# google/zopfli

Hardware: AMD Instinct MI355X
Metric: input MB/s at numiterations=15 (gzip, bit-exact vs reference) (higher is better)
Workload: dtype u8 (f32/f64 cost DP); 1 GPU; class-T synthetic (text-like, the enwik8 stand-in) 100000000 B per GPU, numiterations=15, blocksplitting=0, gzip, BASELINE configs[1]; total_bytes=100000000, master_blocks=100, gather=none (one rank)

## Files before the change

### zopfli_amd/csrc/device/drv_build.h

```cpp
#pragma once

constexpr u32 kMatchGrid = 1024;
constexpr u32 kMatchGrid5 = 1536;

extern "C" {
static unsigned SegL(u64 total_positions) {
  if (Knobs().seg_l_set) return Knobs().seg_l;
  return total_positions <= (128u << 10) ? 256u : total_positions <= (16u << 20) ? 512u : total_positions <= (48u << 20) ? 1024u : 2048u;
}
static unsigned SegHead(size_t nb) {
  const unsigned v = Knobs().seg_head;
  return v ? v : (nb >= 48 ? 8192u : 0u);
}


static int LayoutBlocks(zmx_ctx* c, const zmx_block* blocks, size_t nb, zmx_tables* t, u64* la_total, u64* max_window) {
  t->nb = nb;
  t->blocks.resize(nb);
  t->bsize.resize(nb);
  t->store_begin[0].assign(nb, 0);
  t->store_begin[1].assign(nb, 0);
  std::vector<u32> tile_off(nb + 1, 0);
  u64 pos_off = 0, reg_off = 0, la_off = 0, max_l = 0;
  for (size_t b = 0; b < nb; ++b) {
    if (blocks[b].inend < blocks[b].instart || blocks[b].inend > c->insize) {
      return FailMsg("zmx_tables_build: block outside the resident input");
    }
    BlockDesc& d = t->blocks[b];
    d.instart = blocks[b].instart;
    d.inend = blocks[b].inend;
    d.ws = d.instart > ZMX_WINDOW ? d.instart - ZMX_WINDOW : 0;
    if (!c->seg_starts.empty()) {
      const size_t k = static_cast<size_t>(std::upper_bound(c->seg_starts.begin(), c->seg_starts.end(), d.instart) -
                                           c->seg_starts.begin()) - 1;
      const u64 seg_end = k + 1 < c->seg_starts.size() ? c->seg_starts[k + 1] : c->insize;
      if (d.inend > seg_end) return FailMsg("zmx_tables_build: block spans two input segments (zmx_set_input_segments)");
      d.ws = std::max<u64>(d.ws, c->seg_starts[k]);
    }
    d.pos_off = pos_off;
    d.reg_off = reg_off;
    d.la_off = la_off;
    const u64 B = d.inend - d.instart, L = d.inend - d.ws;
    if (B > 0x7fff0000ull) return FailMsg("zmx_tables_build: block too large (positions are 32-bit)");
    t->bsize[b] = static_cast<u32>(B);
    pos_off += B;
    reg_off += (L + 7) & ~7ull;
    la_off += (B + 1 + 7) & ~7ull;
    max_l = std::max(max_l, L);
    tile_off[b + 1] = tile_off[b] + static_cast<u32>((B + MT - 1) / MT);
  }
  t->total_b = pos_off;
  t->total_l = reg_off;
  t->tile_off = tile_off;
  *la_total = la_off;
  *max_window = max_l;
  return 0;
}

struct ReusePlan {
  bool reuse = false;
  std::vector<u64> src_pos;
  std::vector<u64> link_lo;
  std::vector<u32> tile_list;
};
static ReusePlan PlanReuse(const zmx_ctx* c, const zmx_tables* t, const zmx_tables* parent, const std::vector<uint64_t>& tail_r) {
  const size_t nb = t->nb;
  const u64 pos_off = t->total_b;
  const std::vector<u32>& tile_off = t->tile_off;
  ReusePlan plan;
  bool reuse = parent != nullptr && parent->nb > 0 && (c->h_in != nullptr || tail_r.size() == nb) && parent->d_recs != nullptr &&
               parent->total_b + pos_off < (3ull << 30);
  if (reuse) {
    plan.src_pos.resize(nb);
    plan.link_lo.resize(nb);
    size_t pb = 0;
    for (size_t b = 0; b < nb && reuse; ++b) {
      const BlockDesc& d = t->blocks[b];
      while (pb < parent->nb && parent->blocks[pb].inend < d.inend) ++pb;
      if (pb == parent->nb || d.instart < parent->blocks[pb].instart || d.inend > parent->blocks[pb].inend) {
        reuse = false;
        break;
      }
      const BlockDesc& pd = parent->blocks[pb];
      plan.src_pos[b] = pd.pos_off + (d.instart - pd.instart);
      const u64 B = d.inend - d.instart;
      plan.link_lo[b] = d.inend - d.ws;
      if (B == 0 || d.inend == pd.inend) continue;
      u64 t0 = B > ZMX_MAX_MATCH ? d.inend - ZMX_MAX_MATCH : d.instart;
      const u64 r = c->h_in ? zamd::TailRunStart(c->h_in, d.instart, d.inend) : tail_r[b];
      if (r < t0) t0 = r;
      const u32 tile_first = static_cast<u32>((t0 - d.instart) / MT);
      for (u32 tile = tile_first; tile < tile_off[b + 1] - tile_off[b]; ++tile) {
        plan.tile_list.push_back(tile_off[b] + tile);
      }
      const u64 first_index = d.instart + static_cast<u64>(tile_first) * MT - d.ws;
      plan.link_lo[b] = first_index > ZMX_WINDOW ? first_index - ZMX_WINDOW : 0;
    }
  }
  plan.reuse = reuse;
  return plan;
}

static int TailRuns(zmx_ctx* c, const zmx_tables* t, std::vector<uint64_t>* r) {
  const size_t nb = t->nb;
  std::vector<uint64_t> blocks(2 * nb);
  for (size_t b = 0; b < nb; ++b) {
    blocks[2 * b] = t->blocks[b].instart;
    blocks[2 * b + 1] = t->blocks[b].inend;
  }
  PoolScope tmp(c);
  uint64_t* d_blocks = nullptr;
  uint64_t* d_r = nullptr;
  HIPCHK(tmp.Upload(&d_blocks, blocks.data(), 2 * nb, "d_blocks"));
  HIPCHK(tmp.AllocT(&d_r, nb, "d_r"));
  TailRunParams P;
  P.in = c->d_in;
  P.blocks = d_blocks;
  P.r = d_r;
  hipLaunchKernelGGL(k_tail_runs, dim3(static_cast<unsigned>(nb)), dim3(64), 0, c->stream, P);
  KCHK(c, "k_tail_runs");
  r->resize(nb);
  HIPCHK(hipMemcpyAsync(r->data(), d_r, nb * sizeof(uint64_t), hipMemcpyDeviceToHost, c->stream));
  HIPCHK(hipStreamSynchronize(c->stream));
  return 0;
}

static int AllocTableArrays(zmx_ctx* c, zmx_tables* t, u64 la_off) {
  const size_t nb = t->nb;
  const u64 pos_off = t->total_b;
  const u64 reg_off = t->total_l;
  const std::vector<u32>& tile_off = t->tile_off;
  HIPCHK(PoolAlloc(c, &t->d_blocks, nb));
  HIPCHK(PoolAlloc(c, &t->d_tile_off, nb + 1));
  HIPCHK(PoolAlloc(c, &t->d_same16, reg_off));
  HIPCHK(PoolAlloc(c, &t->d_links, reg_off));
  HIPCHK(PoolAlloc(c, &t->d_recs, pos_off * 8));
  HIPCHK(PoolAlloc(c, &t->d_la, la_off));
  HIPCHK(PoolAlloc(c, &t->d_store[0], pos_off));
  HIPCHK(PoolAlloc(c, &t->d_store[1], pos_off));
  t->run = RunLayout(nb);
  HIPCHK(PoolAlloc(c, &t->d_runin, t->run.in_bytes));
  HIPCHK(PoolAlloc(c, &t->d_runout, t->run.out_bytes));
  HIPCHK(c->pool.PinnedTake(&t->h_runin, t->run.in_bytes, &t->h_runin_cap));
  HIPCHK(c->pool.PinnedTake(&t->h_runout, t->run.out_bytes, &t->h_runout_cap));
  HIPCHK(hipMemsetAsync(t->run.stats(t->d_runout), 0, RunLayout::stats_and_flags_bytes(), c->stream));
  HIPCHK(PoolAlloc(c, &t->d_dph, pos_off));
  HIPCHK(PoolAlloc(c, &t->d_block_edges, nb));
  t->badpos_words = pos_off / 32 + 4;
  HIPCHK(PoolAlloc(c, &t->d_badpos, t->badpos_words));
  HIPCHK(PoolAlloc(c, &t->d_code_base, nb));
  HIPCHK(PoolAlloc(c, &t->d_wtab, nb * ZMX_WTAB));
  HIPCHK(PoolAlloc(c, &t->d_badcodes, nb * 40));
  HIPCHK(PoolAlloc(c, &t->d_counters, 48));
  HIPCHK(hipMemcpyAsync(t->d_blocks, t->blocks.data(), nb * sizeof(BlockDesc), hipMemcpyHostToDevice, c->stream));
  HIPCHK(hipMemcpyAsync(t->d_tile_off, tile_off.data(), (nb + 1) * sizeof(u32), hipMemcpyHostToDevice, c->stream));
  HIPCHK(hipMemsetAsync(t->run.flags(t->d_runout), 0, RunLayout::kFlags * sizeof(u32), c->stream));
  return 0;
}

struct MatchBuild {
// ... 231 lines not shown
    HIPCHK(hipMemsetAsync(t->d_counters, 0, 48 * sizeof(u32), c->stream));
    if (LaunchMatch(c, t, mk, m, t->d_pool, t->pool_cap, tile_off[nb], nullptr, Knobs().prof) != 0) return -1;
    u32 counters[2] = {0, 0};
    HIPCHK(hipMemcpyAsync(counters, t->d_counters, sizeof(counters), hipMemcpyDeviceToHost, c->stream));
    HIPCHK(hipStreamSynchronize(c->stream));
    match_positions += static_cast<double>(pos_off);
    if (m.d_m5stats) {
      const size_t m5_waves = static_cast<size_t>(kMatchGrid5) * (M5_THREADS / 64);
      std::vector<unsigned long long> ws(2 * m5_waves);
      HIPCHK(hipMemcpy(ws.data(), m.d_m5stats, ws.size() * sizeof(unsigned long long), hipMemcpyDeviceToHost));
      m5_lane_iters = m5_iters = 0;
      for (size_t w = 0; w < m5_waves; ++w) { m5_lane_iters += static_cast<double>(ws[2 * w]); m5_iters += static_cast<double>(ws[2 * w + 1]); }
    }
    if (counters[1] & 2u) {
      u32 dbg[8] = {0};
      HIPCHK(hipMemcpy(dbg, t->d_counters + 32, sizeof(dbg), hipMemcpyDeviceToHost));
      char buf[320];
      std::snprintf(buf, sizeof(buf), "zmx_tables_build: k_match5's wave loop did not end (state %08x xd %u curd %u bestlen %u limit %u nlink %u eqd %u "
                    "li %u idx %u same %u cur %u bestdist %u)", dbg[0], dbg[1], dbg[2], dbg[3] & 0xffffu, dbg[3] >> 16, dbg[4] & 0xffffu, dbg[4] >> 16,
                    dbg[5], dbg[6] & 0xffffu, dbg[6] >> 16, dbg[7] & 0xffffu, dbg[7] >> 16);
      return FailFault(buf);
    }
    if ((counters[1] & 1u) == 0) break;
    if (per_pos >= 256) return FailMsg("zmx_tables_build: change-point pool overflow");
    per_pos *= 8;
  }
  {
    HIPCHK(hipEventRecord(c->ev[2], c->stream));
    HIPCHK(hipEventSynchronize(c->ev[2]));
    float ms_hash = 0, ms_match = 0;
    HIPCHK(hipEventElapsedTime(&ms_hash, c->ev[0], c->ev[1]));
    HIPCHK(hipEventElapsedTime(&ms_match, c->ev[1], c->ev[2]));
    zmx_stats& ts = zamd::ThreadStats();
    ts.match[0] += ms_match * 1e-3;
    ts.match[1] += ms_hash * 1e-3;
    ts.match[2] += 1;
    ts.match[3] += reuse ? static_cast<double>(plan.tile_list.size()) * MT : match_positions;
    if (m.skip_any && !reuse) {
      ts.match5[0] += m5_lane_iters;
      ts.match5[1] += m5_iters;
      ts.match5[2] += m.skip_positions;
    }
    if (Knobs().prof && !reuse) {
      unsigned long long hc[2] = {0, 0};
      HIPCHK(hipMemcpy(hc, t->d_counters + 4, sizeof(hc), hipMemcpyDeviceToHost));
      const double pos = static_cast<double>(pos_off);
      std::fprintf(stderr, "%s: %.2f ms for %.0f positions: %.1f chain hits per "
                   "position, %.1f of 64 lanes with a hit per wave-loop iteration; %.1f SIMD cycles per hit (2.4 GHz, 1024 SIMDs)\n", mk == 5 || mk == 0 ? "k_match5 / k_match2 (hits = entries touched)" : "k_match2", ms_match, pos,
                   static_cast<double>(hc[0]) / pos, static_cast<double>(hc[0]) / static_cast<double>(hc[1] ? hc[1] : 1),
                   ms_match * 1e-3 * 2.4e9 * 1024 / static_cast<double>(hc[0] ? hc[0] : 1));
      if (mk != 5) {
        int wgs = 0;
        if (Knobs().match_filter) HIPCHK(hipOccupancyMaxActiveBlocksPerMultiprocessor(&wgs, k_match2<false, true>, M2_THREADS, 0));
        else HIPCHK(hipOccupancyMaxActiveBlocksPerMultiprocessor(&wgs, k_match2<false, false>, M2_THREADS, 0));
        std::fprintf(stderr, "k_match2: %d workgroups of %u threads resident per CU; positions handed out %s\n", wgs, M2_THREADS,
                     m.d_est ? "by k_hits' estimate, longest first" : "in ascending order");
      }
    }
  }
  return 0;
}

static int BuildDpRows(zmx_ctx* c, zmx_tables* t) {
  const size_t nb = t->nb;
  const std::vector<u32>& tile_off = t->tile_off;
  RowScanParams rp;
  rp.blocks = t->d_blocks;
  rp.recs = t->d_recs;
  rp.dph = t->d_dph;
  rp.block_edges = t->d_block_edges;
  rp.codeless = !Knobs().run_codes && SegL(t->total_b) != 0 ? 1u : 0u;
  hipLaunchKernelGGL(k_rowscan, dim3(static_cast<unsigned>(nb)), dim3(1024), 0, c->stream, rp);
  KCHK(c, "k_rowscan");
  t->block_edges.resize(nb);
  HIPCHK(hipMemcpyAsync(t->block_edges.data(), t->d_block_edges, nb * sizeof(u64), hipMemcpyDeviceToHost, c->stream));
  HIPCHK(hipStreamSynchronize(c->stream));
  {
    const u64 env_mb = Knobs().code_budget_mb;
    const u64 budget = (env_mb ? env_mb * (1ull << 20) : static_cast<u64>(c->code_budget)) / sizeof(u16);
    std::vector<u64> code_base(nb, 0);
    u64 cur = 0;
    for (size_t b = 0; b < nb; ++b) {
      if (t->block_edges[b] > 0xffff0000ull) return FailMsg("zmx_tables_build: block too large (DP row offsets are 32-bit)");
      code_base[b] = cur;
      cur += ((t->block_edges[b] + DP_PIECE - 1) & ~static_cast<u64>(DP_PIECE - 1)) + DP_PIECE;
    }
    if (cur > budget && nb > 1) {
      return FailTooLarge("zmx_tables_build: the batch needs more room for its DP edges than ZOPFLI_AMD_CODE_BUDGET_MB allows");
    }
    HIPCHK(PoolAlloc(c, &t->d_codes, cur + 2048));
    HIPCHK(hipMemcpyAsync(t->d_code_base, code_base.data(), nb * sizeof(u64), hipMemcpyHostToDevice, c->stream));
    CodeParams kp;
    kp.blocks = t->d_blocks;
    kp.tile_off = t->d_tile_off;
    kp.nb_total = static_cast<u32>(nb);
    kp.recs = t->d_recs;
    kp.pool = t->d_pool;
    kp.dph = t->d_dph;
    kp.codes = t->d_codes;
    kp.code_base = t->d_code_base;
    if (tile_off[nb]) hipLaunchKernelGGL(k_codes, dim3(tile_off[nb]), dim3(256), 0, c->stream, kp);
    KCHK(c, "k_codes");
    t->win_off.assign(nb + 1, 0);
    for (size_t b = 0; b < nb; ++b) t->win_off[b + 1] = t->win_off[b] + (t->bsize[b] + 31) / 32 + 1;
    HIPCHK(PoolAlloc(c, &t->d_winflag, t->win_off[nb]));
    HIPCHK(PoolAlloc(c, &t->d_winroff, t->win_off[nb]));
    HIPCHK(PoolAlloc(c, &t->d_wmeta, (static_cast<size_t>(t->win_off[nb]) + 2) * D5_WM));
    HIPCHK(PoolAlloc(c, &t->d_win_off, nb + 1));
    HIPCHK(hipMemcpyAsync(t->d_win_off, t->win_off.data(), (nb + 1) * sizeof(u32), hipMemcpyHostToDevice, c->stream));
    MkDescParams mp;
    mp.blocks = t->d_blocks;
    mp.dph = t->d_dph;
    mp.wmeta = t->d_wmeta;
    mp.winroff = t->d_winroff;
    mp.win_off = t->d_win_off;
    mp.winflag = t->d_winflag;
    u32 max_b = 1;
    for (size_t b = 0; b < nb; ++b) max_b = std::max(max_b, t->bsize[b]);
    hipLaunchKernelGGL(k_mkdesc, dim3((max_b + 255) / 256, static_cast<unsigned>(nb)), dim3(256), 0, c->stream, mp);
    KCHK(c, "k_mkdesc");
    HIPCHK(hipStreamSynchronize(c->stream));
  }
  return 0;
}

static int BuildChainTasks(zmx_ctx* c, zmx_tables* t) {
  const size_t nb = t->nb;
  const u32 L = SegL(t->total_b), warm = Knobs().seg_warm;
  const u32 head = std::max(SegHead(nb), L);
  t->task_off.assign(nb + 1, 0);
  t->tasks.clear();
  for (size_t b = 0; b < nb; ++b) {
    const u32 B = t->bsize[b];
    const u32 n = (L == 0 || B < head + L) ? 1u : 1u + (B - head) / L;
    for (u32 s = 0; s < n; ++s) {
      SegTask k;
      k.block = static_cast<u32>(b);
      k.pout = s == 0 ? 0u : head + (s - 1) * L;
      k.q = s == 0 ? 0u : k.pout - std::min(warm, k.pout);
      k.pend = s + 1 == n ? B + 1 : head + s * L;
      t->tasks.push_back(k);
    }
    t->task_off[b + 1] = static_cast<u32>(t->tasks.size());
  }
  const size_t nt = t->tasks.size();
  HIPCHK(PoolAlloc(c, &t->d_tasks, nt));
  HIPCHK(PoolAlloc(c, &t->d_task_off, nb + 1));
  HIPCHK(PoolAlloc(c, &t->d_lvl, nt));
  HIPCHK(PoolAlloc(c, &t->d_entry, nt));
  HIPCHK(PoolAlloc(c, &t->d_exit, nt));
  HIPCHK(PoolAlloc(c, &t->d_mid, nt));
  HIPCHK(PoolAlloc(c, &t->d_chk, nt));
  HIPCHK(PoolAlloc(c, &t->d_over, nt * SEG_OVER));
  HIPCHK(PoolAlloc(c, &t->d_redo, 4 + nt * 4));
  HIPCHK(hipMemcpyAsync(t->d_tasks, t->tasks.data(), nt * sizeof(SegTask), hipMemcpyHostToDevice, c->stream));
  HIPCHK(hipMemcpyAsync(t->d_task_off, t->task_off.data(), (nb + 1) * sizeof(u32), hipMemcpyHostToDevice, c->stream));
  HIPCHK(hipMemsetAsync(t->run.stats(t->d_runout), 0, RunLayout::kStats * sizeof(u32), c->stream));
  const u32 cut_depth = Knobs().seg_cuts;
  if (cut_depth && nt) {
    PoolScope tmp(c);
    u32* d_found = nullptr;
    u32* d_wide = nullptr;
    HIPCHK(tmp.AllocT(&d_found, 2, "d_found"));
    HIPCHK(tmp.AllocT(&d_wide, nt, "d_wide"));
    HIPCHK(hipMemsetAsync(d_found, 0, 2 * sizeof(u32), c->stream));
    HIPCHK(hipMemsetAsync(d_wide, 0, nt * sizeof(u32), c->stream));
    CutParams cp;
    cp.blocks = t->d_blocks;
    cp.dph = t->d_dph;
    cp.tasks = t->d_tasks;
    cp.depth = cut_depth;
    cp.warm = warm;
    cp.found = d_found;
    cp.wide = d_wide;
    hipLaunchKernelGGL(k_cutpoints, dim3(static_cast<unsigned>(nt)), dim3(64), 0, c->stream, cp);
    KCHK(c, "k_cutpoints");
    u32 found[2] = {0, 0};
    std::vector<u32> wide(nt);
    HIPCHK(hipMemcpyAsync(found, d_found, sizeof(found), hipMemcpyDeviceToHost, c->stream));
    HIPCHK(hipMemcpyAsync(wide.data(), d_wide, nt * sizeof(u32), hipMemcpyDeviceToHost, c->stream));
    HIPCHK(hipMemcpyAsync(t->tasks.data(), t->d_tasks, nt * sizeof(SegTask), hipMemcpyDeviceToHost, c->stream));
    HIPCHK(hipStreamSynchronize(c->stream));
    size_t merged = 0;
    std::vector<SegTask> kept;
    kept.reserve(nt);
    std::vector<u32> off(nb + 1, 0);
    for (size_t b = 0; b < nb; ++b) {
      for (u32 k = t->task_off[b]; k < t->task_off[b + 1]; ++k) {
        if (k > t->task_off[b] && wide[k]) {
          kept.back().pend = t->tasks[k].pend;
          ++merged;
        } else {
          kept.push_back(t->tasks[k]);
        }
      }
      off[b + 1] = static_cast<u32>(kept.size());
    }
    t->merged_tasks = merged;
    if (merged) {
      t->tasks.swap(kept);
      t->task_off.swap(off);
      HIPCHK(hipMemcpyAsync(t->d_tasks, t->tasks.data(), t->tasks.size() * sizeof(SegTask), hipMemcpyHostToDevice, c->stream));
      HIPCHK(hipMemcpyAsync(t->d_task_off, t->task_off.data(), (nb + 1) * sizeof(u32), hipMemcpyHostToDevice, c->stream));
      HIPCHK(hipStreamSynchronize(c->stream));
    }
    if (Knobs().prof) {
      std::fprintf(stderr, "k_cutpoints: %u of %zu tasks start at a cut point, %.1f positions before their first owned one on average; "
                   "%zu tasks merged into their predecessors (long-run material in the warm-up stretch), %zu tasks left\n",
                   found[0], nt, found[0] ? static_cast<double>(found[1]) / found[0] : 0.0, merged, t->tasks.size());
    }
  }
  return 0;
}

static int BuildWorkgroupLists(zmx_ctx* c, zmx_tables* t) {
  const size_t nb = t->nb;
  const size_t ntk = t->tasks.size();
  std::vector<u32> kind(ntk, 0);
  if (ntk) {
    PoolScope tmp(c);
    u32* d_kind = nullptr;
    HIPCHK(tmp.AllocT(&d_kind, ntk, "d_kind"));
    TaskKindParams kp;
    kp.tasks = t->d_tasks;
    kp.blocks = t->d_blocks;
    kp.winflag = t->d_winflag;
    kp.win_off = t->d_win_off;
    kp.kind = d_kind;
    hipLaunchKernelGGL(k_taskkind, dim3(static_cast<unsigned>(ntk)), dim3(64), 0, c->stream, kp);
    KCHK(c, "k_taskkind");
    HIPCHK(hipMemcpyAsync(kind.data(), d_kind, ntk * sizeof(u32), hipMemcpyDeviceToHost, c->stream));
    HIPCHK(hipStreamSynchronize(c->stream));
  }
  std::vector<u32> wg, wg_runs;
  for (int pass = 0; pass < 2; ++pass) {
    for (size_t b = 0; b < nb; ++b) {
      const u32 a0 = t->task_off[b], a1 = t->task_off[b + 1];
      std::vector<u32> grp[2];
      for (u32 k = a0; k < a1; ++k) grp[kind[k] ? 1 : 0].push_back(k);
      for (int kd = 0; kd < 2; ++kd) {
        std::vector<u32>& dst = kd ? wg_runs : wg;
        for (size_t i = 0; i < grp[kd].size(); i += D5_WG) {
          const bool has_head = i == 0 && !grp[kd].empty() && grp[kd][0] == a0;
          if ((pass == 0) != has_head) continue;
          for (u32 w = 0; w < D5_WG; ++w) dst.push_back(i + w < grp[kd].size() ? grp[kd][i + w] : SEG_NONE);
        }
      }
    }
  }
  t->n_wg = static_cast<u32>(wg.size() / D5_WG);
  t->n_wg_runs = static_cast<u32>(wg_runs.size() / D5_WG);
  wg.insert(wg.end(), wg_runs.begin(), wg_runs.end());
  HIPCHK(PoolAlloc(c, &t->d_wg_tasks, wg.size() + 4));
  if (!wg.empty()) HIPCHK(hipMemcpyAsync(t->d_wg_tasks, wg.data(), wg.size() * sizeof(u32), hipMemcpyHostToDevice, c->stream));
  HIPCHK(hipStreamSynchronize(c->stream));
  return 0;
}

static int BuildTraceSegments(zmx_ctx* c, zmx_tables* t) {
  const size_t nb = t->nb;
  t->seg_off.assign(nb + 1, 0);
  for (size_t b = 0; b < nb; ++b) t->seg_off[b + 1] = t->seg_off[b] + (t->bsize[b] + TS_SEG - 1) / TS_SEG;
  HIPCHK(PoolAlloc(c, &t->d_seg_off, nb + 1));
  HIPCHK(PoolAlloc(c, &t->d_extab, static_cast<size_t>(t->seg_off[nb]) * GS_STATES));
  HIPCHK(PoolAlloc(c, &t->d_seginfo, t->seg_off[nb]));
  HIPCHK(hipMemcpyAsync(t->d_seg_off, t->seg_off.data(), (nb + 1) * sizeof(u32), hipMemcpyHostToDevice, c->stream));
  HIPCHK(hipStreamSynchronize(c->stream));
  return 0;
}

static void FillTableParams(zmx_tables* t, bool with_dp) {
  const u32 nb = static_cast<u32>(t->nb);
  GreedySegParams& gp = t->params.greedy;
  gp.blocks = t->d_blocks;
  gp.seg_off = t->d_seg_off;
  gp.nb = nb;
  gp.recs = t->d_recs;
  gp.hist_out = t->run.hist(t->d_runout);
  gp.nsym_out = t->run.nsym(t->d_runout);
  gp.extab = t->d_extab;
  gp.seginfo = t->d_seginfo;
  if (!with_dp) return;
  const RunLayout& run = t->run;
  WtabParams& wp = t->params.wtab;
  wp.cost = run.cost(t->d_runin);
  wp.mincost = run.mincost(t->d_runin);
  wp.wtab = t->d_wtab;
  wp.badcodes = t->d_badcodes;
  wp.stats = t->run.stats(t->d_runout);
  BadScanParams& bp = t->params.badscan;
  bp.blocks = t->d_blocks;
  bp.tile_off = t->d_tile_off;
  bp.nb_total = nb;
  bp.dph = t->d_dph;
  bp.codes = t->d_codes;
  bp.code_base = t->d_code_base;
  bp.badcodes = t->d_badcodes;
  bp.badpos = t->d_badpos;
  Dp4Params& cp = t->params.dp;
  cp.blocks = t->d_blocks;
  cp.dph = t->d_dph;
  cp.cost = wp.cost;
  cp.mincost = wp.mincost;
  cp.codes = t->d_codes;
  cp.code_base = t->d_code_base;
  cp.block_edges = t->d_block_edges;
  cp.wtab = t->d_wtab;
  cp.la = t->d_la;
  cp.badpos = t->d_badpos;
  cp.tasks = t->d_tasks;
  cp.task_off = t->d_task_off;
  cp.lvl = t->d_lvl;
  cp.entry = t->d_entry;
  cp.exit = t->d_exit;
  cp.chk = t->d_chk;
  cp.over = t->d_over;
  cp.wmax = run.wmax(t->d_runin);
  cp.tiemask = run.tiemask(t->d_runin);
  cp.stats = t->run.stats(t->d_runout);
  cp.wg_tasks = t->d_wg_tasks;
  cp.redo_count = t->d_redo;
  cp.redo_wg = t->d_redo + 4;
  cp.flags = t->run.flags(t->d_runout);
  cp.wmeta = t->d_wmeta;
  cp.winroff = t->d_winroff;
  cp.winflag = t->d_winflag;
  cp.win_off = t->d_win_off;
  TraceSegParams& tp = t->params.trace;
  tp.blocks = t->d_blocks;
  tp.seg_off = t->d_seg_off;
  tp.nb_total = nb;
  tp.recs = t->d_recs;
  tp.pool = t->d_pool;
  tp.la = t->d_la;
  tp.slot = t->run.slot(t->d_runin);
  tp.store0 = t->d_store[0];
  tp.store1 = t->d_store[1];
  tp.hist_out = t->run.hist(t->d_runout);
  tp.nsym_out = t->run.nsym(t->d_runout);
  tp.flags = t->run.flags(t->d_runout);
  tp.extab = t->d_extab;
  tp.seginfo = t->d_seginfo;
}

static int BuildTables(zmx_ctx* c, const zmx_block* blocks, size_t nb, zmx_tables* t, zmx_tables* parent, bool with_dp) {
  const int mk = MatchKernel();
  t->matches_only = !with_dp;
  u64 la_off = 0, max_l = 0;
  if (const int rc = LayoutBlocks(c, blocks, nb, t, &la_off, &max_l)) return rc;
  if (nb == 0) return 0;
  std::vector<uint64_t> tail_r;
  if (parent != nullptr && c->h_in == nullptr) {
    if (const int rc = TailRuns(c, t, &tail_r)) return rc;
  }
  const ReusePlan plan = PlanReuse(c, t, parent, tail_r);
  if (const int rc = AllocTableArrays(c, t, la_off)) return rc;
  MatchBuild m(c);
  if (const int rc = BuildHashLinks(c, t, mk, max_l, plan, m)) return rc;
  if (const int rc = BuildMatchRecords(c, t, parent, mk, max_l, plan, m)) return rc;
  if (with_dp) {
    if (const int rc = BuildDpRows(c, t)) return rc;
    if (const int rc = BuildChainTasks(c, t)) return rc;
    if (const int rc = BuildWorkgroupLists(c, t)) return rc;
  }
  if (const int rc = BuildTraceSegments(c, t)) return rc;
  FillTableParams(t, with_dp);
  return 0;
}

int zmx_tables_build(zmx_ctx* c, const zmx_block* blocks, size_t nblocks, zmx_tables** out) {
  return zmx_tables_build_from(c, nullptr, blocks, nblocks, out);
}

static int BuildTablesEntry(zmx_ctx* c, zmx_tables* parent, const zmx_block* blocks, size_t nblocks, bool with_dp, zmx_tables** out) {
  DEVICE_ENTRY(c->device);
  zmx_tables* t = new zmx_tables();
  g_last_oom = false;
  const int rc = BuildTables(c, blocks, nblocks, t, parent, with_dp);
  if (rc) {
    zmx_tables_free(c, t);
    return rc == -1 && g_last_oom && nblocks > 1 ? kTooLarge : rc;
  }
  *out = t;
  return 0;
}

int zmx_tables_build_matches(zmx_ctx* c, const zmx_block* blocks, size_t nblocks, zmx_tables** out) {
  return BuildTablesEntry(c, nullptr, blocks, nblocks, false, out);
}

int zmx_tables_build_from(zmx_ctx* c, zmx_tables* parent, const zmx_block* blocks, size_t nblocks, zmx_tables** out) {
  if (parent != nullptr && CheckTables("zmx_tables_build_from", parent, zamd::kUntrimmed) != 0) return -1;
  return BuildTablesEntry(c, parent, blocks, nblocks, true, out);
}
}
```

### zopfli_amd/csrc/device/drv_squeeze.h

```cpp
#pragma once

extern "C" {
int zmx_lz77_greedy(zmx_ctx* c, zmx_tables* t, int slot, uint32_t* nsym, uint32_t* hist) {
  if (const int rc = CheckTables("zmx_lz77_greedy", t, zamd::kUntrimmed)) return rc;
  if (t->nb == 0) return 0;
  if (slot != 0 && slot != 1) return FailMsg("zmx_lz77_greedy: slot must be 0 or 1");
  DEVICE_ENTRY(c->device);
  GreedySegParams gp = t->params.greedy;
  gp.store = t->d_store[slot];
  const unsigned nseg = t->seg_off[t->nb];
  if (nseg) hipLaunchKernelGGL(k_greedy_exits, dim3(nseg), dim3(GS_THREADS), 0, c->stream, gp);
  KCHK(c, "k_greedy_exits");
  hipLaunchKernelGGL(k_greedy_link, dim3(static_cast<unsigned>(t->nb)), dim3(64), 0, c->stream, gp);
  KCHK(c, "k_greedy_link");
  if (nseg) hipLaunchKernelGGL(k_greedy_emit, dim3(nseg), dim3(64), 0, c->stream, gp);
  KCHK(c, "k_greedy_emit");
  HIPCHK(hipMemcpyAsync(nsym, t->run.nsym(t->d_runout), t->nb * sizeof(u32), hipMemcpyDeviceToHost, c->stream));
  HIPCHK(hipMemcpyAsync(hist, t->run.hist(t->d_runout), t->nb * ZMX_HIST * sizeof(u32), hipMemcpyDeviceToHost, c->stream));
  HIPCHK(hipStreamSynchronize(c->stream));
  for (size_t b = 0; b < t->nb; ++b) t->store_begin[slot][b] = 0;
  t->h_hist.assign(hist, hist + t->nb * ZMX_HIST);
  t->have_hist = true;
  return 0;
}

static void RunInfo(const double* cost, const u32* hist, u32 B, float* wmax_out, u32* tiemask_out, float* est_out,
                    double mincost = 0.0, bool* below_mincost = nullptr) {
  const double* ll = cost;
  const double* d = cost + ZMX_NUM_LL;
  auto lbits = [](int s) { return s < 265 || s == 285 ? 0 : (s - 261) / 4; };
  auto dbits = [](int s) { return s < 4 ? 0 : s / 2 - 1; };
  double w[256 + 29 * 30];
  int n = 0;
  for (int i = 0; i < 256; ++i) w[n++] = ll[i];
  for (int ls = 257; ls <= 285; ++ls)
    for (int ds = 0; ds < 30; ++ds) w[n++] = (static_cast<double>(lbits(ls) + dbits(ds)) + ll[ls]) + d[ds];
  double wmax = 0;
  for (int i = 0; i < n; ++i) wmax = std::max(wmax, w[i]);
  if (below_mincost) {
    bool any = false;
    for (int i = 256; i < n; ++i) any |= w[i] < mincost;
    *below_mincost = any;
  }
  u32 mask = 0;
  for (int i = 0; i < n; ++i) {
    if (!(w[i] > 0)) continue;
    int x;
    const double fr = std::frexp(w[i], &x);
    const uint64_t m = static_cast<uint64_t>(std::ldexp(fr, 53));
    x -= 53;
    {
      auto run27 = [](uint64_t y) {
        uint64_t a = y & (y >> 1);
        a &= a >> 2; a &= a >> 4; a &= a >> 8;
        return (a & (a >> 11)) != 0;
      };
      const uint64_t mask53 = (1ull << 53) - 1;
      if (!run27(~m & mask53) && !run27(m) && (m & ((1ull << 26) - 1)) != 0) continue;
    }
    for (int e = 4; e < 32; ++e) {
      const int sh = -(x + 52 - e);
      uint64_t r;
      if (sh <= 0) {
        if (-sh >= 29) continue;
        r = m << -sh;
      } else if (sh >= 64) {
        continue;
      } else {
        const uint64_t q = m >> sh, rem = m & ((1ull << sh) - 1), half = 1ull << (sh - 1);
        r = q + ((rem > half || (rem == half && (q & 1))) ? 1 : 0);
      }
      if ((r & 0x1fffffffull) == 0x10000000ull) mask |= 1u << e;
    }
  }
  *wmax_out = static_cast<float>(wmax) + 1.0f;
  *tiemask_out = mask;
  double est = 8.0 * B;
  if (hist) {
    est = 0;
    for (int i = 0; i < ZMX_NUM_LL; ++i) est += hist[i] * (ll[i] + (i > 256 ? lbits(i) : 0));
    for (int i = 0; i < 30; ++i) est += hist[ZMX_NUM_LL + i] * (d[i] + dbits(i));
  }
  *est_out = static_cast<float>(est);
}

void zmx_internal_run_info(const double* cost320, float* wmax, uint32_t* tiemask) {
  float est;
  RunInfo(cost320, nullptr, 0, wmax, tiemask, &est);
}

static int ReportSqueezeProf(zmx_tables* t, const double* ksec, const u32* segstats) {
  const size_t nb = t->nb;
  std::vector<u64> pr(nb * ZMX_PROF_N);
  HIPCHK(hipMemcpy(pr.data(), t->d_prof, pr.size() * sizeof(u64), hipMemcpyDeviceToHost));
  double a[ZMX_PROF_N] = {};
  for (size_t b = 0; b < nb; ++b)
    for (unsigned k = 0; k < ZMX_PROF_N; ++k) a[k] += static_cast<double>(pr[b * ZMX_PROF_N + k]);
  std::fprintf(stderr, "squeeze prof: edges %.2f ms chain %.2f ms trace %.2f ms; chain wave busy %.1f cycles/position, "
               "%.0f steps, fast %.1f%% of %.0f positions walked (%zu in the blocks); tasks %u accepted %u re-run "
               "state %u values %u level %u tie %u (%u positions, %u by the lean job)\n",
               ksec[0] * 1e3, ksec[1] * 1e3, ksec[2] * 1e3, a[1] / a[4], a[0],
               100.0 * a[2] / (a[2] + a[3] + 1e-9), a[4], t->total_b, segstats[0], segstats[1], segstats[2],
               segstats[6], segstats[3], segstats[4], segstats[5], segstats[7]);
  {
    double mx = 0, hd = 0;
    for (size_t b = 0; b < nb; ++b) { mx = std::max(mx, static_cast<double>(pr[b * ZMX_PROF_N + 7])); hd = std::max(hd, static_cast<double>(pr[b * ZMX_PROF_N + 8])); }
    std::fprintf(stderr, "  k_dp5_spec: longest task %.0f cycles, longest head task %.0f cycles; %.1f%% of the positions walked by the integer step (cycles per position there: fetch issue %.1f, fetch wait %.1f, gather + chain %.1f)\n", mx, hd, 100.0 * a[10] / (a[4] + 1e-9), a[11] / (a[10] + 1e-9), a[12] / (a[10] + 1e-9), a[13] / (a[10] + 1e-9));
  }
  std::fprintf(stderr, "  k_dp5_spec integer windows, cycles per position: class decision %.1f, waiting for the prefetched record and codes %.1f, prefetch issue %.1f\n",
               a[20] / (a[10] + 1e-9), a[21] / (a[10] + 1e-9), a[22] / (a[10] + 1e-9));
  std::fprintf(stderr, "  k_dp5_spec windows: integer %.1f%% of positions at %.0f cycles each, class 1 in doubles %.1f%% at %.0f, class 2 %.1f%% at %.0f, generic %.1f%% at %.0f\n",
               100.0 * a[28] / (a[4] + 1e-9), a[24] / (a[28] + 1e-9), 100.0 * a[29] / (a[4] + 1e-9), a[25] / (a[29] + 1e-9),
               100.0 * a[30] / (a[4] + 1e-9), a[26] / (a[30] + 1e-9), 100.0 * a[31] / (a[4] + 1e-9), a[27] / (a[31] + 1e-9));
  std::fprintf(stderr, "  k_dp5_spec generic windows, cycles each: shortcut %.0f (%.0f of them), run row integer %.0f (%.0f), run row doubles %.0f (%.0f), other row %.0f (%.0f), window header %.0f (%.0f)\n",
               a[32] / (a[33] + 1e-9), a[33], a[34] / (a[35] + 1e-9), a[35], a[36] / (a[37] + 1e-9), a[37], a[38] / (a[39] + 1e-9), a[39], a[40] / (a[41] + 1e-9), a[41]);
  std::fprintf(stderr, "  k_dp5_spec positions: run interior %.0f in unrolled windows, %.0f in loops with room, %.0f with checks; general step: %.0f run rows, %.0f other rows; class 2: %.0f rows that reach register 2\n",
               a[42], a[43], a[44], a[45], a[46], a[47]);
  {
    const double gen = a[51] - a[49] - a[50] - a[52];
    std::fprintf(stderr, "  k_dp5_spec generic windows, cycles: headers %.3g, run stretches: whole windows %.3g (%.0f per position), others %.3g (%.0f); stretches of other rows %.3g (%.0f); the general step %.3g (%.0f per position incl. shortcuts)\n",
                 a[48], a[49], a[49] / (a[42] + 1e-9), a[50], a[50] / (a[43] + a[44] + 1e-9), a[52], a[52] / (a[53] + 1e-9), gen, gen / (a[45] + a[46] + a[33] + 1e-9));
  }
  const char* nm[5] = {"32", "16", "8", "8 (two registers)", "generic"};
  for (int i = 0; i < 5; ++i)
    std::fprintf(stderr, "  path %-18s %5.1f%% of positions, %6.1f cycles/position\n", nm[i], 100.0 * a[6 + 2 * i] / a[4],
                 a[5 + 2 * i] / (a[6 + 2 * i] + 1e-9));
  for (int w = 0; w < 2; ++w)
    std::fprintf(stderr, "  producer wave %d, cycles/step: walk %.0f ring %.0f tiles %.0f barrier %.0f\n", w + 1,
                 a[16 + 8 * w] / a[0], a[17 + 8 * w] / a[0], a[18 + 8 * w] / a[0], a[19 + 8 * w] / a[0]);
  return 0;
}

static int TraceAndCollect(zmx_ctx* c, zmx_tables* t, const TraceSegParams& tp, const int32_t* slot, uint32_t* nsym,
                           uint32_t* hist, bool timing, u32* segstats, const char* who) {
  const size_t nb = t->nb;
  const unsigned nblk = static_cast<unsigned>(nb);
  const unsigned nseg = t->seg_off[nb];
  if (nseg) hipLaunchKernelGGL(k_trace_exits, dim3(nseg), dim3(TS_THREADS), 0, c->stream, tp);
  KCHK(c, "k_trace_exits");
  hipLaunchKernelGGL(k_trace_link, dim3(nblk), dim3(64), 0, c->stream, tp);
  KCHK(c, "k_trace_link");
  if (nseg) hipLaunchKernelGGL(k_trace_emit, dim3(nseg), dim3(64), 0, c->stream, tp);
  KCHK(c, "k_trace_emit");
  if (timing) HIPCHK(hipEventRecord(c->ev[3], c->stream));
  HIPCHK(hipMemcpyAsync(t->h_runout, t->d_runout, t->run.out_bytes, hipMemcpyDeviceToHost, c->stream));
  HIPCHK(hipStreamSynchronize(c->stream));
  const u32* o_flags = t->run.flags(t->h_runout);
  std::memcpy(hist, t->run.hist(t->h_runout), nb * ZMX_HIST * sizeof(u32));
  std::memcpy(nsym, t->run.nsym(t->h_runout), nb * sizeof(u32));
  std::memcpy(segstats, t->run.stats(t->h_runout), RunLayout::kStats * sizeof(u32));
  if (o_flags[1]) {
    char buf[128];
    std::snprintf(buf, sizeof(buf), "%s: device consistency flags 0x%x", who, o_flags[1]);
    return FailFault(buf);
  }
  t->h_hist.assign(hist, hist + nb * ZMX_HIST);
  t->have_hist = true;
  for (size_t b = 0; b < nb; ++b) t->store_begin[slot[b]][b] = t->bsize[b] - nsym[b];
  return 0;
}

static void LaunchSpec(hipStream_t stream, unsigned grid, bool run_tasks, const Dp4Params& p) {
  const dim3 g(grid), b(64 * D5_WG);
  if (run_tasks) {
    if (p.prof) hipLaunchKernelGGL((k_dp5_spec<true, 2, true>), g, b, 0, stream, p);
    else hipLaunchKernelGGL((k_dp5_spec<false, 2, true>), g, b, 0, stream, p);
  } else {
    if (p.prof) hipLaunchKernelGGL((k_dp5_spec<true, 4, false>), g, b, 0, stream, p);
    else hipLaunchKernelGGL((k_dp5_spec<false, 4, false>), g, b, 0, stream, p);
  }
}
static void LaunchFix(hipStream_t stream, unsigned nblk, const Dp4Params& p) {
  const dim3 b(64 * (D3_NB + 2));
  if (p.prof) hipLaunchKernelGGL(k_dp4_fix<true>, dim3(nblk), b, 0, stream, p);
  else hipLaunchKernelGGL(k_dp4_fix<false>, dim3(nblk), b, 0, stream, p);
}

int zmx_squeeze_run(zmx_ctx* c, zmx_tables* t, const double* cost, const double* mincost, const int32_t* slot,
                    uint32_t* nsym, uint32_t* hist) {
  if (const int rc = CheckTables("zmx_squeeze_run", t, zamd::SqueezeRunNeeds(t ? t->nb : 0))) return rc;
  if (t->nb == 0) return 0;
  DEVICE_ENTRY(c->device);
  for (size_t b = 0; b < t->nb; ++b) {
    if (slot[b] != 0 && slot[b] != 1) return FailMsg("zmx_squeeze_run: slot must be 0 or 1");
  }
  const size_t nb = t->nb;
  const zamd::DeviceKnobs& knobs = Knobs();
  bool any_below_mincost = false;
  {
    const RunLayout& run = t->run;
    float* wmax = run.wmax(t->h_runin);
    u32* tiemask = run.tiemask(t->h_runin);
    float* est = run.est(t->h_runin);
    std::memcpy(run.cost(t->h_runin), cost, nb * ZMX_HIST * sizeof(double));
    std::memcpy(run.mincost(t->h_runin), mincost, nb * sizeof(double));
    std::memcpy(run.slot(t->h_runin), slot, nb * sizeof(int));
    const u32* hh = t->have_hist ? t->h_hist.data() : nullptr;
    std::vector<char> below(nb, 0);
    zamd::ParallelFor(nb, [&](size_t b) {
      bool bad = false;
      RunInfo(cost + b * ZMX_HIST, hh ? hh + b * ZMX_HIST : nullptr, t->bsize[b], &wmax[b], &tiemask[b], &est[b], mincost[b], &bad);
      below[b] = bad ? 1 : 0;
    });
    for (size_t b = 0; b < nb; ++b) any_below_mincost |= below[b] != 0;
  }
  HIPCHK(hipMemcpyAsync(t->d_runin, t->h_runin, t->run.in_bytes, hipMemcpyHostToDevice, c->stream));
  if (knobs.prof && !t->d_prof) HIPCHK(PoolAlloc(c, &t->d_prof, nb * ZMX_PROF_N));
  if (t->d_prof) HIPCHK(hipMemsetAsync(t->d_prof, 0, nb * ZMX_PROF_N * sizeof(u64), c->stream));
  Dp4Params cp = t->params.dp;
  cp.est_bits = t->squeeze_runs == 0 ? t->run.est(t->d_runin) : nullptr;
  cp.prof = t->d_prof;
  cp.mid = knobs.seg_mid ? t->d_mid : nullptr;
  cp.level_scale = knobs.seg_scale;
  cp.debug = knobs.seg_debug;
  cp.fix_lean_min = knobs.fix_lean;
  cp.int_path = knobs.int_path;
  cp.chain_fast = knobs.shortcut_chain;
  const bool scan_bad = any_below_mincost;
  if (scan_bad || !t->badpos_clean) HIPCHK(hipMemsetAsync(t->d_badpos, 0, t->badpos_words * sizeof(u32), c->stream));
  t->badpos_clean = !scan_bad;
  double ksec[3] = {0, 0, 0};
  const bool timing = KernelTiming();
  {
    const unsigned nblk = static_cast<unsigned>(nb);
    const unsigned tiles = t->tile_off[nb];
    const unsigned ntask = t->task_off[nb];
    if (timing) HIPCHK(hipEventRecord(c->ev[0], c->stream));
    hipLaunchKernelGGL(k_wtab, dim3(nblk), dim3(256), 0, c->stream, t->params.wtab);
    KCHK(c, "k_wtab");
    if (tiles && scan_bad) hipLaunchKernelGGL(k_badscan, dim3(tiles), dim3(256), 0, c->stream, t->params.badscan);
    KCHK(c, "k_badscan");
    if (timing) HIPCHK(hipEventRecord(c->ev[1], c->stream));
    {
      if (t->n_wg_runs) {
        HIPCHK(hipEventRecord(c->ev2[0], c->stream));
        HIPCHK(hipStreamWaitEvent(c->stream2, c->ev2[0], 0));
        Dp4Params cr = cp;
        cr.task0 = t->n_wg;
        LaunchSpec(c->stream2, t->n_wg_runs, true, cr);
        HIPCHK(hipGetLastError());
        HIPCHK(hipEventRecord(c->ev2[1], c->stream2));
      }
      if (t->n_wg) {
        LaunchSpec(c->stream, t->n_wg, false, cp);
        HIPCHK(hipGetLastError());
      }
      if (t->n_wg_runs) HIPCHK(hipStreamWaitEvent(c->stream, c->ev2[1], 0));
      if (GuardOn()) HIPCHK(hipStreamSynchronize(c->stream2));
      KCHK(c, "k_dp5_spec");
    }
    if (ntask > nblk) {
      hipLaunchKernelGGL(k_dpcheck, dim3(ntask), dim3(64), 0, c->stream, cp);
      KCHK(c, "k_dpcheck");
      for (int pass = 0; pass < knobs.seg_redo; ++pass) {
        hipLaunchKernelGGL(k_dpscan, dim3(nblk), dim3(64), 0, c->stream, cp);
        KCHK(c, "k_dpscan");
        Dp4Params c2 = cp;
        c2.redo_pass = 1;
        c2.est_bits = nullptr;
        LaunchSpec(c->stream, ntask, t->n_wg_runs != 0, c2);
        KCHK(c, "k_dp5_spec");
        hipLaunchKernelGGL(k_dpcheck, dim3(ntask), dim3(64), 0, c->stream, cp);
        KCHK(c, "k_dpcheck");
      }
      LaunchFix(c->stream, nblk, cp);
      KCHK(c, "k_dp4_fix");
    }
    if (timing) HIPCHK(hipEventRecord(c->ev[2], c->stream));
  }
  u32 segstats[RunLayout::kStats];
  if (const int rc = TraceAndCollect(c, t, t->params.trace, slot, nsym, hist, timing, segstats, "zmx_squeeze_run")) return rc;
  for (int i = 0; i < 3 && timing; ++i) {
    float ms = 0;
    HIPCHK(hipEventElapsedTime(&ms, c->ev[i], c->ev[i + 1]));
    ksec[i] += ms * 1e-3;
  }
  ++t->squeeze_runs;
  {
    zmx_stats& ts = zamd::ThreadStats();
    for (int i = 0; i < 3; ++i) ts.kernel_seconds[i] += ksec[i];
    ts.squeeze_launches += 1;
    for (int i = 0; i < 7; ++i) ts.seg[i] += segstats[i];
    ts.seg[7] += static_cast<double>(t->total_b);
  }
  if (t->d_prof) return ReportSqueezeProf(t, ksec, segstats);
  return 0;
}

int zmx_trace_length_arrays(zmx_ctx* c, zmx_tables* t, size_t nblocks, const uint16_t* const* length_arrays,
                            const size_t* entries, const int32_t* slot, uint32_t* nsym, uint32_t* hist) {
  if (const int rc = CheckTables("zmx_trace_length_arrays", t, zamd::kWithDp)) return rc;
  if (const int rc = Refused(zamd::CheckLengthArrays("zmx_trace_length_arrays", t->nb, [&](size_t b) { return size_t{t->bsize[b]}; },
                                                     nblocks, length_arrays, entries, slot))) return rc;
  const size_t nb = t->nb;
  if (nb == 0) return 0;
  DEVICE_ENTRY(c->device);
  const BlockDesc& last = t->blocks[nb - 1];
  std::vector<u16> rows(last.la_off + ((static_cast<u64>(t->bsize[nb - 1]) + 1 + 7) & ~7ull), 0);
  for (size_t b = 0; b < nb; ++b) std::memcpy(rows.data() + t->blocks[b].la_off, length_arrays[b], entries[b] * sizeof(u16));
  HIPCHK(hipMemcpy(t->d_la, rows.data(), rows.size() * sizeof(u16), hipMemcpyHostToDevice));
  int* h_slot = t->run.slot(t->h_runin);
  std::memcpy(h_slot, slot, nb * sizeof(int));
  HIPCHK(hipMemcpyAsync(t->run.slot(t->d_runin), h_slot, nb * sizeof(int), hipMemcpyHostToDevice, c->stream));
  HIPCHK(hipMemsetAsync(t->run.flags(t->d_runout), 0, RunLayout::kFlags * sizeof(u32), c->stream));
  u32 segstats[RunLayout::kStats];
  const int rc = TraceAndCollect(c, t, t->params.trace, slot, nsym, hist, false, segstats, "zmx_trace_length_arrays");
  if (rc) (void)hipMemsetAsync(t->run.flags(t->d_runout), 0, RunLayout::kFlags * sizeof(u32), c->stream);
  return rc;
}
}
```

### zopfli_amd/csrc/device/drv_tables.h

```cpp
#pragma once

struct RunLayout {
  static constexpr size_t kStats = 8, kFlags = 4;
  size_t in_cost = 0, in_mincost = 0, in_wmax = 0, in_tiemask = 0, in_est = 0, in_slot = 0, in_bytes = 0;
  size_t out_hist = 0, out_nsym = 0, out_stats = 0, out_flags = 0, out_bytes = 0;
  RunLayout() = default;
  explicit RunLayout(size_t nb) {
    in_mincost = in_cost + nb * ZMX_HIST * sizeof(double);
    in_wmax = in_mincost + nb * sizeof(double);
    in_tiemask = in_wmax + nb * sizeof(float);
    in_est = in_tiemask + nb * sizeof(u32);
    in_slot = in_est + nb * sizeof(float);
    in_bytes = in_slot + nb * sizeof(int);
    out_nsym = out_hist + nb * ZMX_HIST * sizeof(u32);
    out_stats = out_nsym + nb * sizeof(u32);
    out_flags = out_stats + kStats * sizeof(u32);
    out_bytes = out_flags + kFlags * sizeof(u32);
  }
  double* cost(unsigned char* in) const { return reinterpret_cast<double*>(in + in_cost); }
  double* mincost(unsigned char* in) const { return reinterpret_cast<double*>(in + in_mincost); }
  float* wmax(unsigned char* in) const { return reinterpret_cast<float*>(in + in_wmax); }
  u32* tiemask(unsigned char* in) const { return reinterpret_cast<u32*>(in + in_tiemask); }
  float* est(unsigned char* in) const { return reinterpret_cast<float*>(in + in_est); }
  int* slot(unsigned char* in) const { return reinterpret_cast<int*>(in + in_slot); }
  u32* hist(unsigned char* out) const { return reinterpret_cast<u32*>(out + out_hist); }
  u32* nsym(unsigned char* out) const { return reinterpret_cast<u32*>(out + out_nsym); }
  u32* stats(unsigned char* out) const { return reinterpret_cast<u32*>(out + out_stats); }
  u32* flags(unsigned char* out) const { return reinterpret_cast<u32*>(out + out_flags); }
  static constexpr size_t stats_and_flags_bytes() { return (kStats + kFlags) * sizeof(u32); }
};

struct TableParams {
  GreedySegParams greedy;
  WtabParams wtab;
  BadScanParams badscan;
  Dp4Params dp;
  TraceSegParams trace;
};

struct zmx_tables {
  size_t nb = 0;
  std::vector<BlockDesc> blocks;
  std::vector<u32> bsize;
  std::vector<u32> store_begin[2];
  size_t total_b = 0, total_l = 0;
  BlockDesc* d_blocks = nullptr;
  u32* d_tile_off = nullptr;
  u16* d_same16 = nullptr;
  ushort4* d_links = nullptr;
  bool links_partial = false;
  size_t merged_tasks = 0;
  bool matches_only = false;
  bool trimmed = false;
  u32* d_recs = nullptr;
  u32* d_pool = nullptr;
  u32 pool_cap = 0;
  u16* d_la = nullptr;
  u32* d_store[2] = {nullptr, nullptr};
  uint2* d_dph = nullptr;
  u64* d_block_edges = nullptr;
  u32* d_badpos = nullptr;
  size_t badpos_words = 0;
  bool badpos_clean = false;
  u64* d_code_base = nullptr;
  u16* d_codes = nullptr;
  double* d_wtab = nullptr;
  u32* d_badcodes = nullptr;
  u32* d_seg_off = nullptr;
  u32* d_extab = nullptr;
  uint2* d_seginfo = nullptr;
  std::vector<u32> seg_off;
  std::vector<u64> block_edges;
  std::vector<u32> tile_off;
  u32* d_counters = nullptr;
  RunLayout run;
  unsigned char* d_runin = nullptr;
  unsigned char* d_runout = nullptr;
  unsigned char* h_runin = nullptr;
  unsigned char* h_runout = nullptr;
  size_t h_runin_cap = 0, h_runout_cap = 0;
  TableParams params = {};
  u64* d_prof = nullptr;
  std::vector<SegTask> tasks;
  std::vector<u32> task_off;
  SegTask* d_tasks = nullptr;
  u32* d_task_off = nullptr;
  u32* d_wg_tasks = nullptr;
  u32 n_wg = 0;
  u32 n_wg_runs = 0;
  u32* d_wmeta = nullptr;
  u32* d_winroff = nullptr;
  u32* d_winflag = nullptr;
  u32* d_win_off = nullptr;
  std::vector<u32> win_off;
  float* d_lvl = nullptr;
  SegSnap* d_entry = nullptr;
  SegSnap* d_exit = nullptr;
  SegSnap* d_mid = nullptr;
  SegCheck* d_chk = nullptr;
  u16* d_over = nullptr;
  u32* d_redo = nullptr;
  std::vector<u32> h_hist;
  bool have_hist = false;
  u32 squeeze_runs = 0;
  std::vector<std::vector<u32>> probe_recs;
  std::vector<u32> probe_pool;
  bool probe_pool_ready = false;
};

extern "C" {
static void ReleaseTableArrays(zmx_ctx* c, zmx_tables* t, bool keep_stores) {
  auto rel = [&](auto*&... p) { ((PoolFree(c, p), p = nullptr), ...); };
  rel(t->d_blocks, t->d_tile_off, t->d_same16, t->d_links, t->d_recs, t->d_pool, t->d_la, t->d_dph, t->d_block_edges);
  rel(t->d_badpos, t->d_code_base, t->d_codes, t->d_wtab, t->d_badcodes, t->d_seg_off, t->d_extab, t->d_seginfo);
  rel(t->d_counters, t->d_prof, t->d_tasks, t->d_task_off, t->d_wg_tasks, t->d_wmeta, t->d_runin, t->d_runout);
  rel(t->d_winroff, t->d_winflag, t->d_win_off, t->d_lvl, t->d_entry, t->d_exit, t->d_mid, t->d_chk, t->d_over, t->d_redo);
  PinnedGive(c, &t->h_runin, t->h_runin_cap);
  PinnedGive(c, &t->h_runout, t->h_runout_cap);
  t->params = TableParams{};
  if (!keep_stores) rel(t->d_store[0], t->d_store[1]);
}

void zmx_tables_free(zmx_ctx* c, zmx_tables* t) {
  if (!t) return;
  DeviceGuard dev_guard(c ? c->device : 0);
  if (c && c->stream2) (void)hipStreamSynchronize(c->stream2);
  ReleaseTableArrays(c, t, false);
  delete t;
}

int zmx_tables_trim(zmx_ctx* c, zmx_tables* t) {
  if (!t) return 0;
  DEVICE_ENTRY(c->device);
  HIPCHK(hipStreamSynchronize(c->stream));
  HIPCHK(hipStreamSynchronize(c->stream2));
  ReleaseTableArrays(c, t, true);
  t->trimmed = true;
  return 0;
}

static int Refused(const std::string& refusal) { return refusal.empty() ? 0 : FailMsg(refusal); }
static int CheckTables(const char* who, const zmx_tables* t, zamd::TableNeeds needs) {
  return Refused(zamd::CheckTables(who, t != nullptr, t && t->trimmed, t && t->matches_only, needs));
}
static int CheckBlock(const char* who, const zmx_tables* t, size_t block) {
  return Refused(zamd::CheckBlock(who, t->nb, block));
}
static int CheckStoreRef(const char* who, const zmx_tables* t, size_t block, int slot, size_t nsym) {
  return Refused(zamd::CheckStoreRef(who, t->nb, block, slot, nsym,
                                     [&] { return static_cast<size_t>(t->bsize[block] - t->store_begin[slot][block]); }));
}
}
```

### zopfli_amd/csrc/device/zmx_dp4.h

```cpp
#pragma once

#define D3_RELAX_K(CS, LT, WV, K)                                            \
  {                                                                          \
    const double old_ = (double)(CS);                                        \
    const double nc_ = (WV) + cj;                                            \
    LT = nc_ < old_ ? (K) : LT;                                              \
    CS = (float)fmin(nc_, old_);                                             \
  }

#define D3_ROT32()                                                           \
  {                                                                          \
    if (reach < 64) {                    \
      c[0] = __uint_as_float(__builtin_amdgcn_permlane32_swap(__float_as_uint(c[0]), __float_as_uint(1e30f), false, false)[1]); \
      l[0] = __builtin_amdgcn_permlane32_swap(l[0], 0u, false, false)[1];    \
    } else {                                                                 \
      d3_rot32(c, l, lane);                                                  \
    }                                                                        \
    reach = reach >= 32 ? reach - 32 : 0;                                    \
  }

#define D4_TRACK_MAX() { vmax = fmaxf(vmax, c[0] < 1e29f ? c[0] : 0.0f); }

#define D3_RETIRE32(WB)                                                      \
  {                                                                          \
// ... 78 lines not shown
    W.pf_a = dbase[nxt];
    W.pf_wa = badpos[(pos_off + nxt) >> 5];
  }
  W.pf_sel ^= 1;
  W.pf_base = W.base + 64;
  G.kend = act ? (dh.y & 0xffffu) : 0u;
  G.roff = dh.x;
  G.offend = G.roff + G.kend;
  G.m_short = __ballot(act && ((dh.y >> 16) & 1u) != 0);
  G.m_r1 = __ballot(G.kend + (lane & 31u) >= 64u);
  G.m_bad = G.m_short | __ballot(G.kend + (lane & 31u) >= 128u) | (G.m_r1 & 0xffffffffull) |
            __ballot(act && ((bw >> ((pos_off + cur) & 31u)) & 1u) != 0);
  W.have_group = true;
}

__device__ __forceinline__ D3Step d3_next(D3Walk& W, D3Group& G, const uint2* dbase, const u32* badpos, u32 pos_off,
                                          u32 B, u32 lane) {
  D3Step S;
  if (W.bubbles) {
    S.base = W.base; S.q = 0; S.n = 0; S.a_cur = 0;
    S.event = W.bubbles == 2 ? D3_EV_BUBBLE : D3_EV_PRIME;
    --W.bubbles;
    if (S.event == D3_EV_PRIME) {
      if (!W.have_group && W.base <= B) { d3_load_group(W, G, dbase, badpos, pos_off, B, lane); W.q = 0; }
      S.a_cur = rdlane_u32(G.roff, 0) & ~(DP_PIECE - 1);
    }
    return S;
  }
  if (!W.have_group) { d3_load_group(W, G, dbase, badpos, pos_off, B, lane); W.q = 0; }
  u64 ms = W.q < 64 ? G.m_short & ~((1ull << W.q) - 1) : 0ull;
  if (W.noshort) ms &= ~(1ull << W.q);
  const u32 stop = ms ? (u32)__ffsll((long long)ms) - 1 : 64u;
  const u32 limit = stop < G.navail ? stop : G.navail;
  S.base = W.base; S.q = W.q; S.n = 0; S.a_cur = 0;
  if (W.q < limit) {
    S.a_cur = rdlane_u32(G.roff, W.q) & ~(DP_PIECE - 1);
    const u64 fit = __ballot(lane >= W.q && lane < limit && G.offend - S.a_cur <= D3_SPAN);
    S.n = (u32)__popcll(fit);
  }
  if (ms && W.q + S.n == stop) {
    S.event = D3_EV_SHORTCUT;
    W.base = W.base + stop + ZMX_MAX_MATCH;
    W.noshort = true;
    W.have_group = false;
    W.bubbles = 2;
  } else if (W.q + S.n == G.navail) {
    S.event = D3_EV_GROUP_END;
    W.base += 64;
    if (S.n) W.noshort = false;
    W.have_group = false;
  } else {
    S.event = D3_EV_NONE;
    W.q += S.n;
    W.noshort = false;
  }
  return S;
}

__device__ __forceinline__ void d3_rot32_u(u32 (&x)[6], u32 fresh, bool lo) {
  u32 t = x[0];
#pragma unroll
  for (int s = 0; s < 5; ++s) {
    const auto r = __builtin_amdgcn_permlane32_swap(t, x[s + 1], false, false);
    x[s] = lo ? r[1] : r[0];
    t = r[1];
  }
  const auto r = __builtin_amdgcn_permlane32_swap(t, fresh, false, false);
  x[5] = r[1];
}

__device__ __forceinline__ void d3_rot32(float (&c)[6], u32 (&l)[6], u32 lane) {
  const bool lo = lane < 32;
  u32 cu[6];
#pragma unroll
  for (int s = 0; s < 6; ++s) cu[s] = __float_as_uint(c[s]);
  d3_rot32_u(cu, __float_as_uint(1e30f), lo);
#pragma unroll
  for (int s = 0; s < 6; ++s) c[s] = __uint_as_float(cu[s]);
  d3_rot32_u(l, 0u, lo);
}

__device__ __forceinline__ bool d3_fast(u32 end, u64 m_bad, u32 p0) {
  return p0 + 8 <= end && (p0 & 31u) <= 24u && ((u32)(m_bad >> p0) & 255u) == 0;
}

__device__ __forceinline__ float wave_max_f32(float v) {
#pragma unroll
  for (int o = 32; o >= 1; o >>= 1) v = fmaxf(v, __shfl_xor(v, o, 64));
  return v;
}
__device__ __forceinline__ float wave_min_f32(float v) {
#pragma unroll
  for (int o = 32; o >= 1; o >>= 1) v = fminf(v, __shfl_xor(v, o, 64));
  return v;
}

__device__ __forceinline__ SegCheck d4_check(const SegSnap* E, const SegSnap* N, u32 lane) {
  bool bad = E->base != N->base || E->noshort != N->noshort || E->skip != N->skip;
  bool badv = false;
  double dl[6];
  bool fin[6];
  float vmin = 3e38f;
#pragma unroll
  for (int s = 0; s < 6; ++s) {
    const u32 i = 64u * s + lane;
    const float ec = E->c[i], nc = N->c[i];
    const bool ef = ec < 1e29f, nf = nc < 1e29f;
    bad |= ef != nf || E->l[i] != N->l[i];
    fin[s] = ef && nf;
    dl[s] = (double)ec - (double)nc;
    if (nf) vmin = fminf(vmin, nc);
  }
  const u32 ref = (u32)__builtin_amdgcn_readfirstlane((int)(E->skip < 32u ? E->skip : 0u));
  const u32 lo = (u32)__builtin_amdgcn_readlane((int)(u32)__double_as_longlong(dl[0]), ref);
  const u32 hi = (u32)__builtin_amdgcn_readlane((int)(u32)(__double_as_longlong(dl[0]) >> 32), ref);
  const double d0 = __longlong_as_double((long long)(((u64)hi << 32) | lo));
  const bool fin0 = __builtin_amdgcn_readlane(fin[0] ? 1 : 0, ref) != 0;
#pragma unroll
  for (int s = 0; s < 6; ++s) badv |= fin[s] && dl[s] != d0;
  SegCheck r;
  r.d = d0;
  r.vmin = wave_min_f32(vmin);
  r.match = (__any(bad) || !fin0) ? 0u : __any(badv) ? 2u : 1u;
  return r;
}

struct Dp4Params {
  const BlockDesc* blocks;
  u32 block0;
  u32 task0;
  const uint2* dph;
  const double* cost;
  const double* mincost;
  const u16* codes;
  const u64* code_base;
  const u64* block_edges;
  const double* wtab;
  u16* la;
  u64* prof;
  const u32* badpos;
  const SegTask* tasks;
  const u32* task_off;
  float* lvl;
  const float* est_bits;
  SegSnap* entry;
  SegSnap* exit;
  SegSnap* mid;
  SegCheck* chk;
  const float* wmax;
  const u32* tiemask;
  u32* stats;
  float level_scale;
  const u32* wg_tasks;
  const u32* wmeta;
  const u32* winroff;
  const u32* winflag;
  const u32* win_off;
  int debug;
  u16* over;
  u32* redo_count;
  u32* redo_wg;
  int int_path;
  int fix_lean_min;
  int redo_pass;
  int chain_fast;
  u32* flags;
};

struct D4Job {
  u32 cell = 0;
  u32 start;
  u32 noshort;
  u32 pout;
  u32 pend;
  u32 la_lo;
  u32 over_lo;
  bool spec;
  bool load;
  float level;
  double delta;
  const SegSnap* init;
  SegSnap* entry;
  SegSnap* exit;
  SegSnap* mid = nullptr;
  u16* over;
};

#define D4_LDS_DECL                                                                                   \
  __shared__ __align__(16) u16 s_ring[DP_FRONT + DP_RING + DP_MIRROR];    \
  __shared__ __align__(16) double s_wtab[ZMX_WTAB];                              \
  __shared__ __align__(16) double s_t1[2][64 * 64];    \
  __shared__ __align__(16) double s_t2[2][32 * 64];         \
  __shared__ uint2 s_tab[D3_NB][64];                                                                  \
   \
                    \
  __shared__ __align__(8) u32 s_desc[3][8];                                                           \
  __shared__ uint2 s_tabc[3][64];                               \
  __shared__ float s_xc[DP_XN];                                                                       \
  __shared__ u16 s_xl[DP_XN];                                                                         \
       \
              \
  __shared__ u32 s_lout[2][128];

template <bool PROF>
__device__ __forceinline__ void d4_run_job(const Dp4Params& P, const D4Job& J, u32 b, const BlockDesc& bd,
                                           u16 (&s_ring)[DP_FRONT + DP_RING + DP_MIRROR], double (&s_wtab)[ZMX_WTAB],
                                           double (&s_t1)[2][64 * 64],
                                           double (&s_t2)[2][32 * 64], uint2 (&s_tab)[D3_NB][64], u32 (&s_desc)[3][8],
                                           uint2 (&s_tabc)[3][64], float (&s_xc)[DP_XN], u16 (&s_xl)[DP_XN],
                                           u32 (&s_lout)[2][128]) {
  const u32 tid = threadIdx.x;
  const u32 wave = (u32)__builtin_amdgcn_readfirstlane((int)(tid >> 6));
  const u32 lane = tid & 63;
  const u32 B = (u32)(bd.inend - bd.instart);
  const uint2* dbase = P.dph + bd.pos_off;
  u16* la = P.la + bd.la_off;
  const u16* rows = P.codes + P.code_base[b];
  const u32 total_pad = (u32)((P.block_edges[b] + DP_PIECE - 1) & ~(u64)(DP_PIECE - 1));
  const double mincost = P.mincost[b];
  const double symbolcost258 = (double)(0 + 0) + P.cost[(u64)b * 320 + 285] + P.cost[(u64)b * 320 + 288];
  const double kInf = __longlong_as_double(0x7ff0000000000000ll);
  const u32 ring_lds = (u32)(unsigned long)(__attribute__((address_space(3))) u16*)s_ring;
  auto ring_w = [&](const u16* slot) -> double {
    return *reinterpret_cast<const double*>(reinterpret_cast<const char*>(s_wtab) + ((u32)*slot & 0x3ff8u));
  };
#define D3_TICK() (PROF ? (u64)__builtin_readcyclecounter() : 0ull)

  if (wave == 0) {
    float c[6];
    u32 l[6];
    u32 reach;
    {
#pragma unroll
      for (int s = 0; s < 6; ++s) {
        const float ec = J.init->c[64u * s + lane];
        c[s] = ec < 1e29f ? (float)((double)ec + J.delta) : 1e30f;
        l[s] = J.init->l[64u * s + lane];
      }
      reach = SEG_CELLS - 1;
    }
    const u32 la_lo = J.la_lo;
    u32 wo = 0;
    u64 t_work = 0, n_fast = 0, n_slow = 0, n_steps = 0;
    u64 tp[5] = {0, 0, 0, 0, 0}, np[5] = {0, 0, 0, 0, 0};

    __syncthreads();
    __syncthreads();
    u32 it = 2;
    uint2 nd = *reinterpret_cast<const uint2*>(s_desc[0]);
    for (;;) {
      const u64 tw0 = PROF ? (u64)__builtin_readcyclecounter() : 0ull;
      u32 dv[6];
      dv[0] = (u32)__builtin_amdgcn_readfirstlane((int)nd.x);
      dv[1] = (u32)__builtin_amdgcn_readfirstlane((int)nd.y);
      nd = *reinterpret_cast<const uint2*>(s_desc[(it - 1) % 3]);
      dv[2] = dv[3] = dv[4] = dv[5] = 0;
      if (!(dv[0] & D3_DESC_CLEAN)) {
#pragma unroll
        for (int i = 2; i < 6; ++i) dv[i] = s_desc[(it - 2) % 3][i];
#pragma unroll
        for (int i = 2; i < 6; ++i) dv[i] = (u32)__builtin_amdgcn_readfirstlane((int)dv[i]);
      }
      D3Step S;
      S.q = dv[0] & 255u; S.n = (dv[0] >> 8) & 255u; S.event = (dv[0] >> 16) & 255u; S.base = dv[1]; S.a_cur = 0;
      const bool last = ((dv[0] >> 24) & 1u) != 0;
      struct { u64 m_r1, m_bad; } G;
      G.m_r1 = ((u64)dv[3] << 32) | dv[2];
      G.m_bad = ((u64)dv[5] << 32) | dv[4];
      const uint2* tabc = s_tabc[(it - 2) % 3];
      const double* t1 = s_t1[it & 1];
      const double* t2 = s_t2[it & 1];
      const u32 send = S.q + S.n;
      const u32 base = S.base;
      u32 p0 = S.q;
      u32 bi = 0;
      if ((dv[0] & D3_DESC_CLEAN) && reach < 64) {
        const u64 tk = D3_TICK();
        double wa[32], wb[32];
#pragma unroll
        for (int u = 0; u < 32; ++u) wa[u] = t1[u * 64 + lane];
#pragma unroll
        for (int u = 0; u < 32; ++u) wb[u] = t1[(32 + u) * 64 + lane];
        u32 lt = 0;
#pragma unroll
        for (int u = 0; u < 32; ++u) {
          const double cj = (double)rdlane_f32(c[0], (u32)u);
          D3_RELAX_K(c[0], lt, wa[u], (u32)(u + 1))
        }
        l[0] = lt ? base + lt : l[0];
        s_lout[it & 1][lane] = l[0];
        c[0] = __uint_as_float(__builtin_amdgcn_permlane32_swap(__float_as_uint(c[0]), __float_as_uint(1e30f), false, false)[1]);
        l[0] = __builtin_amdgcn_permlane32_swap(l[0], 0u, false, false)[1];
        lt = 0;
#pragma unroll
        for (int u = 0; u < 32; ++u) {
          const double cj = (double)rdlane_f32(c[0], (u32)u);
          D3_RELAX_K(c[0], lt, wb[u], (u32)(u + 1))
        }
        l[0] = lt ? base + 32 + lt : l[0];
        n_fast += 64;
        if (PROF) { tp[0] += D3_TICK() - tk; np[0] += 64; }
        s_lout[it & 1][64 + lane] = l[0];
        c[0] = __uint_as_float(__builtin_amdgcn_permlane32_swap(__float_as_uint(c[0]), __float_as_uint(1e30f), false, false)[1]);
        l[0] = __builtin_amdgcn_permlane32_swap(l[0], 0u, false, false)[1];
        reach = 31;
        wo = 0;
        if (PROF) { t_work += (u64)__builtin_readcyclecounter() - tw0; ++n_steps; }
        __syncthreads();
        ++it;
        if (last) break;
        continue;
      }
      for (; p0 < S.q + S.n; ++bi) {
        const u64 tk = D3_TICK();
// ... 223 lines not shown
          issued_end += DP_PIECE;
        }
        if (cur.n) a_prev = cur.a_cur;
      }
      const u64 tk1 = D3_TICK();
      cur.n = 0; cur.event = D3_EV_BUBBLE;
      hb3 = hb2; hc3 = hc2; hb2 = hb1; hc2 = hc1; hc1 = false;
      if (more) {
        cur = d3_next(W, G, dbase, P.badpos + (bd.pos_off >> 5), (u32)(bd.pos_off & 31), B, lane);
        more = W.bubbles || W.base < J.pend;
        if (cur.n) s_tabc[it % 3][lane] = make_uint2(G.roff, G.kend);
        const bool clean = cur.q == 0 && cur.n == 64 && (G.m_r1 | G.m_bad) == 0;
        hb1 = cur.base; hc1 = clean;
        if (lane == 0) {
          u32* d = s_desc[it % 3];
          d[0] = cur.q | (cur.n << 8) | (cur.event << 16) | ((more ? 0u : 1u) << 24) | (clean ? D3_DESC_CLEAN : 0u);
          d[1] = cur.base;
          d[2] = (u32)G.m_r1; d[3] = (u32)(G.m_r1 >> 32);
          d[4] = (u32)G.m_bad; d[5] = (u32)(G.m_bad >> 32);
        }
      } else {
        ++tail;
      }
      const u64 tk2 = D3_TICK();
      __syncthreads();
      if (PROF) { tq[1] += tk1 - tk0; tq[0] += tk2 - tk1; tq[3] += D3_TICK() - tk2; }
      ++it;
    }
    D3_STORE_LA()
#undef D3_STORE_LA
    asm volatile("s_waitcnt vmcnt(0)" ::: "memory");
    if (J.exit && lane == 0) { J.exit->base = W.base; J.exit->noshort = W.noshort ? 1u : 0u; J.exit->skip = 0u; }
    if (PROF && P.prof && lane == 0) {
      u64* o = P.prof + (u64)b * ZMX_PROF_N + 16;
      for (int i = 0; i < 4; ++i) atomicAdd(&o[i], tq[i]);
    }
  } else {
    u64 tq[4] = {0, 0, 0, 0};
    const u32 my = wave - 2;
    __syncthreads();
    u32 it = 1;
    for (;;) {
      const u64 tk0 = D3_TICK();
      u32 dv[6];
      dv[0] = (u32)__builtin_amdgcn_readfirstlane((int)s_desc[(it - 1) % 3][0]);
      dv[2] = dv[3] = dv[4] = dv[5] = 0;
      const bool clean = (dv[0] & D3_DESC_CLEAN) != 0;
      if (!clean) {
#pragma unroll
        for (int i = 2; i < 6; ++i) dv[i] = s_desc[(it - 1) % 3][i];
#pragma unroll
        for (int i = 2; i < 6; ++i) dv[i] = (u32)__builtin_amdgcn_readfirstlane((int)dv[i]);
      }
      const u32 sq = dv[0] & 255u, sn = (dv[0] >> 8) & 255u, sev = (dv[0] >> 16) & 255u;
      const bool last = ((dv[0] >> 24) & 1u) != 0;
      const u64 m_r1 = ((u64)dv[3] << 32) | dv[2], m_bad = ((u64)dv[5] << 32) | dv[4];
      if (sn && sev != D3_EV_BUBBLE && sev != D3_EV_PRIME) {
        const uint2 tc = s_tabc[(it - 1) % 3][lane];
        wave_lds_sync();
        s_tab[my][lane] = make_uint2(((tc.x & (DP_RING - 1)) - lane - 1) * 2u, tc.y);
        wave_lds_sync();
        double* t1 = s_t1[(it - 1) & 1];
        double* t2 = s_t2[(it - 1) & 1];
        const char* ring0 = reinterpret_cast<const char*>(s_ring + DP_FRONT);
        if (clean && D3_NB == 2) {
          const u32 pa = 16u * my, pb = pa + 32u;
          uint2 ta[16], tb[16];
#pragma unroll
          for (int u = 0; u < 16; ++u) { ta[u] = s_tab[my][pa + u]; tb[u] = s_tab[my][pb + u]; }
          double va[16], vb[16];
#pragma unroll
          for (int u = 0; u < 16; ++u) {
            va[u] = ring_w(reinterpret_cast<const u16*>(ring0 + (int)ta[u].x) + lane);
            vb[u] = ring_w(reinterpret_cast<const u16*>(ring0 + (int)tb[u].x) + lane + 32u);
          }
          const u32 da = lane - pa - 1, db = lane + 32u - pb - 1;
#pragma unroll
          for (int u = 0; u < 16; ++u) {
            t1[(pa + u) * 64 + lane] = da - u < ta[u].y ? va[u] : kInf;
            t1[(pb + u) * 64 + lane] = db - u < tb[u].y ? vb[u] : kInf;
          }
          const u64 tk1c = D3_TICK();
          __syncthreads();
          if (PROF) { tq[2] += tk1c - tk0; tq[3] += D3_TICK() - tk1c; }
          ++it;
          if (last) break;
          continue;
        }
        u32 blk = 0;
        for (u32 p0 = sq; p0 < sq + sn; p0 += 8) {
          if (!d3_fast(sq + sn, m_bad, p0)) continue;
          const u32 wl = lane + (p0 & 32u);
          const u32 d0 = wl - p0 - 1;
          if ((p0 & 31u) <= 16u && d3_fast(sq + sn, m_bad, p0 + 8) && ((u32)(m_r1 >> p0) & 0xffffu) == 0) {
            if ((blk++ % D3_NB) == my) {
              uint2 t[16];
#pragma unroll
              for (int u = 0; u < 16; ++u) t[u] = s_tab[my][p0 + u];
              double v0[16];
#pragma unroll
              for (int u = 0; u < 16; ++u) v0[u] = ring_w(reinterpret_cast<const u16*>(ring0 + (int)t[u].x) + wl);
#pragma unroll
              for (int u = 0; u < 16; ++u) t1[(p0 + u) * 64 + lane] = d0 - u < t[u].y ? v0[u] : kInf;
            }
            p0 += 8;
            continue;
          }
          if ((blk++ % D3_NB) != my) continue;
          const bool two = ((u32)(m_r1 >> p0) & 255u) != 0;
          uint2 t[8];
#pragma unroll
          for (int u = 0; u < 8; ++u) t[u] = s_tab[my][p0 + u];
          if (!two) {
            double v0[8];
#pragma unroll
            for (int u = 0; u < 8; ++u) v0[u] = ring_w(reinterpret_cast<const u16*>(ring0 + (int)t[u].x) + wl);
#pragma unroll
            for (int u = 0; u < 8; ++u) t1[(p0 + u) * 64 + lane] = d0 - u < t[u].y ? v0[u] : kInf;
          } else {
            double v0[8], v1[8];
#pragma unroll
            for (int u = 0; u < 8; ++u) {
              const u16* row = reinterpret_cast<const u16*>(ring0 + (int)t[u].x);
              v0[u] = ring_w(row + wl);
              v1[u] = ring_w(row + wl + 64);
            }
#pragma unroll
            for (int u = 0; u < 8; ++u) {
              t1[(p0 + u) * 64 + lane] = d0 - u < t[u].y ? v0[u] : kInf;
              t2[((p0 + u) & 31) * 64 + lane] = d0 - u + 64 < t[u].y ? v1[u] : kInf;
            }
          }
        }
      }
      const u64 tk1 = D3_TICK();
      __syncthreads();
      if (PROF) { tq[2] += tk1 - tk0; tq[3] += D3_TICK() - tk1; }
      ++it;
      if (last) break;
    }
    __syncthreads();
    if (PROF && P.prof && wave == 2 && lane == 0) {
      u64* o = P.prof + (u64)b * ZMX_PROF_N + 24;
      for (int i = 0; i < 4; ++i) atomicAdd(&o[i], tq[i]);
    }
  }
#undef D3_TICK
  __builtin_amdgcn_fence(__ATOMIC_RELEASE, "agent");
  __syncthreads();
  __builtin_amdgcn_fence(__ATOMIC_ACQUIRE, "agent");
}

__global__ __launch_bounds__(64) void k_dpcheck(Dp4Params P) {
  if (blockIdx.x == 0 && threadIdx.x == 0) *P.redo_count = 0;
  const u32 t = P.task0 + blockIdx.x;
  if (P.tasks[t].pout == 0) return;
  const SegCheck r = d4_check(&P.exit[t - 1], &P.entry[t], threadIdx.x);
  if (threadIdx.x == 0) P.chk[t] = r;
}

__device__ __forceinline__ u32 d4_accept(float vmin, double vmax, double delta, double wmax, u32 tiemask) {
  if (delta == 0.0) return 0;
  const int e = (int)((__float_as_uint(vmin) >> 23) & 255u) - 127;
  const double lo = ldexp(1.0, e), hi = ldexp(1.0, e + 1);
  const bool pure = vmin >= 16.0f && vmax + wmax < hi && (double)vmin + delta >= lo && vmax + wmax + delta < hi;
  if (!pure) return 1;
  return ((tiemask >> (e & 31)) & 1u) != 0 ? 2u : 0u;
}

__global__ __launch_bounds__(64) void k_dpscan(Dp4Params P) {
  const u32 b = P.block0 + blockIdx.x;
  const u32 t0 = P.task_off[b], t1 = P.task_off[b + 1];
  const u32 lane = threadIdx.x;
  const double wmax = (double)P.wmax[b] + 1.0;
  const u32 tiemask = P.tiemask[b];
  double carry = 0.0;
  for (u32 c0 = t0 + 1; c0 < t1; c0 += 64) {
    const u32 t = c0 + lane;
    const bool act = t < t1;
    SegCheck ck;
    ck.d = 0.0; ck.vmin = 0.0f; ck.match = 0;
    float vmax = 0.0f;
    if (act) { ck = P.chk[t]; vmax = P.exit[t].vmax; }
    double incl = act ? ck.d : 0.0;
#pragma unroll
    for (int o = 1; o < 64; o <<= 1) {
      const double up = __shfl_up(incl, o, 64);
      if ((int)lane >= o) incl += up;
    }
    const double delta = carry + incl;
    if (act) {
      const bool ok = ck.match == 1 && d4_accept(ck.vmin, (double)vmax, delta, wmax, tiemask) == 0;
      if (!ok && ck.match != 0) {
        const u32 slot = atomicAdd(P.redo_count, 1u);
        u32* wg = P.redo_wg + (u64)slot * 4;
        wg[0] = t; wg[1] = SEG_NONE; wg[2] = SEG_NONE; wg[3] = SEG_NONE;
        P.lvl[t] = (float)((double)P.lvl[t] + delta);
      }
    }
    carry += __shfl(incl, 63, 64);
  }
}

__device__ __forceinline__ void d4_copy_over(const Dp4Params& P, u32 t, u32 B, u16* la) {
  const u32 pend = P.tasks[t].pend;
  if (pend > B) return;
  const u32 stop = P.exit[t].base + P.exit[t].skip;
  const u16* over = P.over + (u64)t * SEG_OVER;
  for (u32 i = threadIdx.x; pend + i < stop && pend + i <= B; i += blockDim.x) la[pend + i] = over[i];
}
```

### zopfli_amd/csrc/device/zmx_dp5.h

```cpp
#pragma once

template <typename T>
__device__ __forceinline__ T* uniform_ptr(T* p) {
  const u64 a = reinterpret_cast<u64>(p);
  const u32 lo = (u32)__builtin_amdgcn_readfirstlane((int)(u32)a), hi = (u32)__builtin_amdgcn_readfirstlane((int)(u32)(a >> 32));
  return reinterpret_cast<T*>(((u64)hi << 32) | lo);
}
typedef u32 d5_u32x4 __attribute__((ext_vector_type(4)));
typedef u32 d5_u32x2 __attribute__((ext_vector_type(2)));
typedef const __attribute__((address_space(4))) d5_u32x4* d5_cdscp;

#define D5_WM 40u
#define D5_WF_CODELESS 0x100u
#define D5_STAGE_BYTES 4352u
#define D5_STAGE_HALF 2176u
struct MkDescParams {
  const BlockDesc* blocks;
  const uint2* dph;
  u32* wmeta;
  u32* winroff;
  const u32* win_off;
  u32* winflag;
};

// ... 881 lines not shown
          for (int s = 0; s < 5; ++s) wv[s] = code_w(cd[s] & 0x3ff8u);
#pragma unroll
          for (int s = 0; s < 5; ++s) {
            const u32 k1 = km1 + 64u * s;
            const double w = k1 < ke ? wv[s] : kInf;
            const double mcl = k1 == 0 ? -kInf : mincost;
            DP_RELAX(c[s], l[s], w, mcl)
          }
        }
        else if (smax < 2) {
#pragma unroll
          for (int s = 0; s < 2; ++s) {
            if ((u32)s <= smax) {
              const u32 k1 = km1 + 64u * s;
              if (k1 < ke) {
                const double w = code_w(rows[ro + k1]);
                const double mcl = k1 == 0 ? -kInf : mincost;
                DP_RELAX(c[s], l[s], w, mcl)
              }
            }
          }
        } else {
          u32 cd[6];
#pragma unroll
          for (int s = 0; s < 6; ++s) {
            const u32 k1 = km1 + 64u * s;
            cd[s] = rows[ro + (k1 < ke ? k1 : 0u)];
          }
#pragma unroll
          for (int s = 0; s < 6; ++s) {
            const u32 k1 = km1 + 64u * s;
            const double w = k1 < ke ? code_w(cd[s]) : kInf;
            const double mcl = k1 == 0 ? -kInf : mincost;
            DP_RELAX(c[s], l[s], w, mcl)
          }
        }
        noshort = false;
        ++n_slow;
        if (fine_) { gq[gk_] += (u64)__builtin_readcyclecounter() - tp0_ + (u64)(__float_as_uint(c[0]) & 0u); ++gq[gk_ + 1]; }
        ++p;
      }
      if (PROF) gt[3] += (u64)__builtin_readcyclecounter() - tg0_ + (u64)(__float_as_uint(c[0]) & 0u);
    }
    if (PROF) { kc[pcls] += (u64)__builtin_readcyclecounter() - tw0; kn[pcls] += n_fast + n_slow - np0; }
    if (jumped) continue;
    {
      const u32 jj = wbase + lane;
      if (lane < 32 && lane >= skip && jj >= la_lo && jj <= B) put_la(jj, (u16)(l[0] ? jj + 1 - l[0] : 0u));
      skip = 0;
      D4_TRACK_MAX()
      D3_ROT32()
      wbase += 32;
    }
  }
#undef D5_PICK16
#undef D5_CHAIN
#undef D5_CHAIN_I
  if (J.la_lo == 1 && lane == 0) la[0] = 0;
  if (J.exit) {
#pragma unroll
    for (int s = 0; s < 6; ++s) {
      J.exit->c[64u * s + lane] = c[s];
      J.exit->l[64u * s + lane] = l[s];
      vmax = fmaxf(vmax, c[s] < 1e29f ? c[s] : 0.0f);
    }
    vmax = wave_max_f32(vmax);
    if (lane == 0) { J.exit->vmax = vmax; J.exit->base = wbase; J.exit->noshort = noshort ? 1u : 0u; J.exit->skip = skip; }
  }
  if (PROF && P.prof && lane == 0) {
    u64* o = P.prof + (u64)b * ZMX_PROF_N;
    atomicAdd(&o[1], (u64)__builtin_readcyclecounter() - t_begin);
    atomicAdd(&o[2], n_fast); atomicAdd(&o[3], n_slow); atomicAdd(&o[4], n_fast + n_slow);
    atomicAdd(&o[5], (u64)__builtin_readcyclecounter() - t_begin); atomicAdd(&o[6], n_fast);
    atomicAdd(&o[14], n_slow);
    atomicAdd(&o[10], n_int);
    for (int i = 0; i < 3; ++i) atomicAdd(&o[20 + i], pw[i]);
    for (int i = 0; i < 4; ++i) { atomicAdd(&o[24 + i], kc[i]); atomicAdd(&o[28 + i], kn[i]); }
    atomicAdd(&o[11], pq[0]); atomicAdd(&o[12], pq[1]); atomicAdd(&o[13], pq[2]);
    for (int i = 0; i < 10; ++i) atomicAdd(&o[32 + i], gq[i]);
    for (int i = 0; i < 6; ++i) atomicAdd(&o[42 + i], gr[i]);
    for (int i = 0; i < 4; ++i) atomicAdd(&o[48 + i], gt[i]);
    atomicAdd(&o[52], go[0]); atomicAdd(&o[53], go[1]);
    const u64 dt = (u64)__builtin_readcyclecounter() - t_begin;
    atomicMax(&o[7], dt);
    if (J.la_lo == 1) atomicAdd(&o[8], dt);
  }
}

struct CutParams {
  const BlockDesc* blocks;
  const uint2* dph;
  SegTask* tasks;
  u32 depth;
  u32 warm;
  u32* found;
  u32* wide;
};

__global__ __launch_bounds__(64) void k_cutpoints(CutParams P) {
  const u32 t = blockIdx.x;
  const SegTask K = P.tasks[t];
  if (K.pout == 0) return;
  const BlockDesc bd = P.blocks[K.block];
  const uint2* dph = P.dph + bd.pos_off;
  const u32 lane = threadIdx.x;
  const u32 lo = K.pout > P.depth + ZMX_MAX_MATCH ? K.pout - P.depth - ZMX_MAX_MATCH : 0u;
  const u32 wlo = K.pout > P.warm ? K.pout - P.warm : 0u;
  const u32 q_min = lo == 0 ? 1u : lo + ZMX_MAX_MATCH;
  u32 carry = 0, best = SEG_NONE;
  bool wide = false;
  for (u32 p0 = lo; p0 < K.pout; p0 += 64) {
    const u32 p = p0 + lane;
    const u32 y = p < K.pout ? dph[p].y : 0u;
    const u32 r = p < K.pout ? p + (y & 0xffffu) : 0u;
    wide |= p >= wlo && (((y >> 16) & 1u) != 0 || (((y >> 17) & 1u) != 0 && (y & 0xffffu) >= 64u));
    u32 incl = wave_scan_max(r);
    incl = incl > carry ? incl : carry;
    const u64 ok = __ballot(p + 1 < K.pout && p + 1 >= q_min && incl <= p + 1);
    if (ok) best = p0 + (63u - (u32)__builtin_clzll(ok)) + 1u;
    carry = rdlane_u32(incl, 63);
  }
  const bool any_wide = __any(wide);
  if (lane == 0) {
    P.wide[t] = best == SEG_NONE && any_wide ? 1u : 0u;
    if (best != SEG_NONE) {
      P.tasks[t].q = best;
      atomicAdd(&P.found[0], 1u);
      atomicAdd(&P.found[1], K.pout - best);
    }
  }
}

struct TaskKindParams {
  const SegTask* tasks;
  const BlockDesc* blocks;
  const u32* winflag;
  const u32* win_off;
  u32* kind;
};
__global__ __launch_bounds__(64) void k_taskkind(TaskKindParams P) {
  const u32 t = blockIdx.x;
  const SegTask K = P.tasks[t];
  const BlockDesc bd = P.blocks[K.block];
  const u32 B = (u32)(bd.inend - bd.instart);
  const u32* wf = P.winflag + P.win_off[K.block];
  const u32 w0 = K.q >> 5, w1 = ((K.pend < B ? K.pend : B) + 31u) >> 5;
  u32 g = 0;
  for (u32 w = w0 + threadIdx.x; w < w1; w += 64) g += (wf[w] & 0xffu) == 0 || (wf[w] & 0xffu) == 3 ? 1u : 0u;
  g = wave_scan_add(g);
  if (threadIdx.x == 63) P.kind[t] = 4u * g >= (w1 - w0) && g >= 4u ? 1u : 0u;
}

#define D5_WG 4u
#define FIX_CH 256u
template <bool PROF, int WAVES, bool RUNS>
__global__ __launch_bounds__(64 * D5_WG, WAVES) void k_dp5_spec(Dp4Params P) {
  __shared__ __align__(16) double s_wtab[ZMX_WTAB];
  __shared__ __align__(16) unsigned char s_buf[D5_WG][D5_STAGE_BYTES];
  __shared__ __align__(8) uint2 s_itab[ZMX_WTAB];
  __shared__ __align__(8) double s_w1[D5_W1];
  __shared__ u8 s_sym1[D5_W1];
  __shared__ __align__(8) uint2 s_ri[D5_WG][32];
  __shared__ __align__(8) uint2 s_rk[RUNS ? D5_WG : 1u][RUNS ? D5_RKN : 1u];
  __shared__ u32 s_rmax;
  const u32 wave = (u32)__builtin_amdgcn_readfirstlane((int)(threadIdx.x >> 6));
  if (P.redo_pass && blockIdx.x >= *P.redo_count) return;
  const u32* wg = (P.redo_pass ? P.redo_wg : P.wg_tasks) + (u64)(P.task0 + blockIdx.x) * D5_WG;
  const u32 t0 = wg[0];
  const u32 b0 = P.tasks[t0].block;
  for (u32 i = threadIdx.x; i < ZMX_WTAB; i += 64 * D5_WG) s_wtab[i] = P.wtab[(u64)b0 * ZMX_WTAB + i];
  if (threadIdx.x == 0) s_rmax = 0;
  __syncthreads();
  d5_build_w1(s_wtab, s_w1, s_sym1);
  auto task_level = [&](u32 tt) -> float {
    const SegTask K = P.tasks[tt];
    float lv = P.est_bits ? P.est_bits[K.block] * ((float)K.q / (float)(u32)(P.blocks[K.block].inend - P.blocks[K.block].instart)) : P.lvl[tt];
    if (!P.redo_pass) lv *= P.level_scale;
    return lv >= 16.0f ? lv : 16.0f;
  };
  D5IntTab IT;
  IT.on = false; IT.lo = 0; IT.span = 0;
  {
    const u32 tl = P.tasks[t0].pout != 0 ? t0 : wg[1];
    if (tl != SEG_NONE && P.int_path) {
      const u32 lb = __float_as_uint(task_level(tl));
      const int e = (int)(lb >> 23) - 127;
      if (e >= 4 && e < 31 && ((P.tiemask[b0] >> (e & 31)) & 1u) == 0) {
        d5_build_inttab(s_wtab, s_itab, s_rmax, e);
        __syncthreads();
        const u32 rm = s_rmax;
        IT.on = true;
        IT.lo = lb & 0x7f800000u;
        IT.span = rm < 0x100000u ? 33u * rm : 0x40000000u;
      }
    }
  }
  const u32 t = wg[wave];
  if (t == SEG_NONE) return;
  const SegTask T = P.tasks[t];
  const BlockDesc bd = P.blocks[T.block];
  const u32 B = (u32)(bd.inend - bd.instart);
  if (B == 0) return;
  D4Job J;
  J.start = T.q & ~31u;
  J.cell = T.q & 31u;
  J.noshort = 0;
  J.pout = T.pout;
  J.pend = T.pend;
  J.load = false;
  J.delta = 0;
  J.init = nullptr;
  J.entry = &P.entry[t];
  J.exit = &P.exit[t];
  J.mid = T.pout != 0 && P.mid != nullptr ? &P.mid[t] : nullptr;
  J.over_lo = T.pend <= B ? T.pend : SEG_NONE;
  J.over = P.over + (u64)t * SEG_OVER;
  if (T.pout == 0) {
    J.spec = false;
    J.la_lo = 1;
    J.level = 0.0f;
  } else {
    J.spec = true;
    J.la_lo = SEG_NONE;
    J.level = task_level(t);
    if (P.est_bits && (threadIdx.x & 63) == 0) P.lvl[t] = J.level;
  }
  d5_run_job<PROF, RUNS>(P, J, T.block, bd, s_wtab, reinterpret_cast<float*>(s_buf[wave]), reinterpret_cast<u16*>(s_buf[wave] + 4u * DP_XN),
                   reinterpret_cast<u16*>(s_buf[wave]), s_itab, IT, s_w1, s_sym1, s_ri[wave], s_rk[RUNS ? wave : 0u]);
}

template <bool PROF>
__global__ __launch_bounds__(64 * (D3_NB + 2)) void k_dp4_fix(Dp4Params P) {
  D4_LDS_DECL
  const u32 b = P.block0 + blockIdx.x;
  const BlockDesc bd = P.blocks[b];
  const u32 B = (u32)(bd.inend - bd.instart);
  if (B == 0) return;
  const u32 t0 = P.task_off[b], t1 = P.task_off[b + 1];
  const u32 lane = threadIdx.x & 63;
  const bool lead = threadIdx.x == 0;
  const double wmax = (double)P.wmax[b] + 1.0;
  const u32 tiemask = P.tiemask[b];
  for (u32 i = threadIdx.x; i < ZMX_WTAB; i += blockDim.x) s_wtab[i] = P.wtab[(u64)b * ZMX_WTAB + i];
  __syncthreads();
  __shared__ __align__(8) double s_w1[D5_W1];
  __shared__ u8 s_sym1[D5_W1];
  __shared__ __align__(8) uint2 s_ri[32];
  d5_build_w1(s_wtab, s_w1, s_sym1);
  u16* la_block = P.la + bd.la_off;
  d4_copy_over(P, t0, B, la_block);
  double delta_prev = 0.0;
  bool rerun_prev = false;
  u32 n_ok = 0, n_state = 0, n_level = 0, n_tie = 0, n_pos = 0, n_values = 0, n_lean = 0, n_mid = 0;
  const u32* winflag = P.winflag + P.win_off[b];
  const u64 cyc0 = __builtin_readcyclecounter();
  u64 cyc_run = 0;
  __shared__ double s_ck_d[FIX_CH], s_dl[FIX_CH];
  __shared__ float s_ck_vmin[FIX_CH], s_vmax[FIX_CH];
  __shared__ u32 s_ck_match[FIX_CH], s_xbase[FIX_CH], s_pend[FIX_CH], s_acc[FIX_CH];
  __shared__ double s_wsum[4], s_dprev;
  __shared__ u32 s_wfail[4];
  static_assert(FIX_CH == 64 * (D3_NB + 2), "the sweep judges a chunk's tasks a thread each");
  for (u32 c0 = t0 + 1; c0 < t1; c0 += FIX_CH) {
  const u32 cn = t1 - c0 < FIX_CH ? t1 - c0 : FIX_CH;
  for (u32 i = threadIdx.x; i < cn; i += blockDim.x) {
    const SegCheck k = P.chk[c0 + i];
    s_ck_d[i] = k.d; s_ck_vmin[i] = k.vmin; s_ck_match[i] = k.match;
    s_vmax[i] = P.exit[c0 + i].vmax;
    s_xbase[i] = P.exit[c0 + i].base + P.exit[c0 + i].skip;
    s_pend[i] = P.tasks[c0 + i].pend;
    s_acc[i] = 0;
    s_dl[i] = 0.0;
  }
  __syncthreads();
  for (u32 t = c0; t < c0 + cn; ++t) {
    if (!rerun_prev) {
      const u32 ti0 = t - c0;
      const u32 i = threadIdx.x;
      const bool act = i >= ti0 && i < cn;
      double incl = act ? s_ck_d[i] : 0.0;
#pragma unroll
      for (int o = 1; o < 64; o <<= 1) {
        const double up = __shfl_up(incl, o, 64);
        if ((int)lane >= o) incl += up;
      }
      if (lane == 63) s_wsum[threadIdx.x >> 6] = incl;
      __syncthreads();
      double before = 0.0;
      for (u32 w = 0; w < (threadIdx.x >> 6); ++w) before += s_wsum[w];
      const double delta_i = delta_prev + before + incl;
      const bool ok_i = act && s_ck_match[i] == 1 && d4_accept(s_ck_vmin[i], (double)s_vmax[i], delta_i, wmax, tiemask) == 0;
      const u64 failm = __ballot(act && !ok_i);
      if (lane == 0) s_wfail[threadIdx.x >> 6] = failm ? (threadIdx.x & ~63u) + (u32)__ffsll((long long)failm) - 1u : 0xffffffffu;
      __syncthreads();
      u32 first_fail = cn;
      for (u32 w = 0; w < (blockDim.x >> 6); ++w) first_fail = s_wfail[w] < first_fail ? s_wfail[w] : first_fail;
      if (act && i < first_fail) { s_acc[i] = 1; s_dl[i] = delta_i; }
      if (first_fail > ti0 && i == first_fail - 1u) s_dprev = delta_i;
      __syncthreads();
      if (first_fail > ti0) { delta_prev = s_dprev; n_ok += first_fail - ti0; }
      t = c0 + first_fail;
      if (t >= c0 + cn) break;
    }
    const u32 ti = t - c0;
    SegCheck ck;
    if (rerun_prev) ck = d4_check(&P.exit[t - 1], &P.entry[t], lane);
    else { ck.d = s_ck_d[ti]; ck.vmin = s_ck_vmin[ti]; ck.match = s_ck_match[ti]; }
    const double delta = delta_prev + ck.d;
    if (lead) s_dl[ti] = delta;
    bool ok = ck.match == 1;
    u32 why = 0;
    if (ok) {
      why = d4_accept(ck.vmin, (double)s_vmax[ti], delta, wmax, tiemask);
      ok = why == 0;
    }
    if (P.debug == 6 && ck.match == 0 && threadIdx.x < 64) {
      const SegSnap* E = &P.exit[t - 1];
      const SegSnap* N = &P.entry[t];
      u32 first = 0xffffffffu;
      for (int s6 = 0; s6 < 6; ++s6) {
        const u32 i = 64u * s6 + lane;
        const bool ef = E->c[i] < 1e29f, nf = N->c[i] < 1e29f;
        if ((ef != nf || E->l[i] != N->l[i]) && i < first) first = i;
      }
      for (int o = 32; o >= 1; o >>= 1) { const u32 v = __shfl_xor(first, o, 64); first = v < first ? v : first; }
      if (lane == 0) {
        const u32 i = first < SEG_CELLS ? first : 0;
        printf("diff b %u t %u pout %u base %u/%u noshort %u/%u skip %u/%u first cell %u: exit c %.4f l %u | entry c %.4f l %u | q %u\n", b, t - t0, P.tasks[t].pout,
               E->base, N->base, E->noshort, N->noshort, E->skip, N->skip, first, (double)E->c[i], E->l[i], (double)N->c[i], N->l[i], P.tasks[t].q);
      }
    }
    if (P.debug == 1 && lead) {
      printf("fix b %u t %u pout %u: match %u d %.6f delta %.6f vmin %.4f vmax %.4f why %u ok %d entry base %u exit-1 base %u\n", b,
             t - t0, P.tasks[t].pout, ck.match, ck.d, delta, (double)ck.vmin, (double)P.exit[t].vmax, why, ok ? 1 : 0,
             P.entry[t].base, P.exit[t - 1].base);
    }
    if (ok) {
      if (lead) s_acc[ti] = 1;
      delta_prev = delta;
      rerun_prev = false;
      ++n_ok;
      continue;
    }
    if (ck.match == 0) ++n_state; else if (ck.match == 2) ++n_values; else if (why == 1) ++n_level; else ++n_tie;
    const SegTask T = P.tasks[t];
    D4Job J;
    J.start = P.exit[t - 1].base;
    J.noshort = P.exit[t - 1].noshort;
    J.pout = 0;
    J.pend = T.pend;
    J.over_lo = SEG_NONE;
    J.spec = false;
    J.load = true;
    J.level = 0.0f;
    J.delta = delta_prev;
    J.init = &P.exit[t - 1];
    J.entry = nullptr;
    J.exit = &P.exit[t];
    J.over = nullptr;
    bool from_mid = false;
    if (ck.match == 1 && why == 1 && P.mid != nullptr) {
      const u32 mb_ = P.mid[t].base;
      if (mb_ != SEG_NONE && mb_ > P.entry[t].base && mb_ < (T.pend < B ? T.pend : B) &&
          d4_accept(ck.vmin, (double)P.mid[t].vmax, delta, wmax, tiemask) == 0) {
        from_mid = true;
        J.start = mb_;
        J.noshort = P.mid[t].noshort;
        J.delta = delta;
        J.init = &P.mid[t];
        ++n_mid;
      }
    }
    J.la_lo = J.start;
    n_pos += (T.pend < B ? T.pend : B) - (J.start < B ? J.start : B);
    const u32 w0 = J.start >> 5, w1 = ((T.pend < B ? T.pend : B) + 31u) >> 5;
    u32 generic = 0, mine = 0, nocodes = 0;
    for (u32 w = w0 + threadIdx.x; w < w1; w += blockDim.x) {
      generic += (winflag[w] & 0xffu) == 0 ? 1u : 0u;
      nocodes |= winflag[w] & D5_WF_CODELESS;
      ++mine;
    }
    const int n_generic = __syncthreads_count((int)generic);
    const int n_major = __syncthreads_count(mine > 0 && 2 * generic >= mine ? 1 : 0);
// ... 50 lines not shown
```

### zopfli_amd/csrc/device/zmx_kernels.h

```cpp
#pragma once
#include <hip/hip_runtime.h>
#include <stdint.h>

#include "zmx_record.h"

typedef unsigned char u8;
typedef unsigned short u16;
typedef unsigned int u32;
typedef unsigned long long u64;

struct BlockDesc {
  u64 instart, inend, ws;
  u64 pos_off;
  u64 reg_off;
  u64 la_off;
};

#define ZMX_WINDOW 32768u
#define ZMX_MAX_MATCH 258u
#define ZMX_MAX_CHAIN_HITS 8192
#define ZMX_NONE16 0xffffu

__device__ __forceinline__ int dev_dist_symbol(u32 d) {
  if (d < 5) return (int)d - 1;
// ... 396 lines not shown
      s_hoff[wid][lane] = (off - off0) | (lit << 16) | ((ovf ? 1u : 0u) << 24);
      if (ovf) {
        s_hpool[wid][lane][0] = zamd::RecPoolOffset(ra.z);
        s_hpool[wid][lane][1] = zamd::RecPoolCount(ra.w);
        s_hthr[wid][lane][0] = 0xffffffffu;
        s_hthr[wid][lane][1] = 0xffffffffu;
      } else {
        const u32 w[6] = {ra.z, ra.w, rb.x, rb.y, rb.z, rb.w};
        u32 t0 = 0, t1 = 0;
#pragma unroll
        for (int e = 0; e < 8; ++e) {
          const u32 v = zamd::RecCpFieldOfWords(w, (u32)e);
          zamd::RecCpThresholdPut(t0, t1, (u32)e, ncpf, v);
          s_hdist[wid][lane][e] = (u16)zamd::RecCpDist(v);
        }
        s_hthr[wid][lane][0] = t0;
        s_hthr[wid][lane][1] = t1;
      }
    }

    u32 q = 0;
    while (q < navail) {
      const u32 off_q = rdlane_u32(off, q);
      const u64 fit = __ballot(act && lane >= q && offend - off_q <= EG_CAP);
      const u32 n = (u32)__popcll(fit);
      const u32 E = rdlane_u32(offend, q + n - 1) - off_q;
      wave_lds_sync();
      for (u32 e = lane; e < (E + 3) / 4; e += 64) reinterpret_cast<u32*>(mark)[e] = 0;
      wave_lds_sync();
      if (lane >= q && lane < q + n && klay != 0) mark[off - off_q] = (u8)(lane + 1);
      wave_lds_sync();
      const u32 rel_q = off_q - off0;
      u32 carry = q + 1;
      u64 ovf_mask = __ballot(lane >= q && lane < q + n && ncpf == zamd::kRecOverflow);
      for (u32 t0 = 0; t0 < E; t0 += 64) {
        const u32 e = t0 + lane;
        const u32 mk = e < E ? (u32)mark[e] : 0u;
        u32 own = wave_scan_max(mk);
        own = own > carry ? own : carry;
        carry = rdlane_u32(own, 63);
        if (e < E) {
          const u32 p = own - 1;
          const u32 h = s_hoff[wid][p];
          const u32 k = e - ((h & 0xffffu) - rel_q) + 1;
          u32 code;
          if (k == 1) {
            code = (1u + ((h >> 16) & 255u)) * 8u;
          } else if (k == 2 || (h >> 24)) {
            code = 0;
          } else {
            const u32 idx = zamd::RecCpThresholdIndex(s_hthr[wid][p][0], s_hthr[wid][p][1], k - 3);
            code = weight_code(k, s_hdist[wid][p][idx]);
          }
          codes[(u64)off_q + e] = (u16)code;
        }
      }
      while (ovf_mask) {
        const u32 p = (u32)__ffsll((long long)ovf_mask) - 1;
        ovf_mask &= ovf_mask - 1;
        const u32 roff_p = rdlane_u32(off, p);
        const u32 ke = rdlane_u32(kend, p);
        const u32 poff = s_hpool[wid][p][0], pn = s_hpool[wid][p][1];
        for (u32 k = 3 + lane; k <= ke; k += 64) {
          const u32 plo = zamd::RecPoolFind(P.pool, poff, pn, k);
          const u32 dist = plo < pn ? zamd::RecPoolDist(P.pool[poff + plo]) : 1u;
          codes[(u64)roff_p + k - 1] = (u16)weight_code(k, dist);
        }
      }
      q += n;
    }
  }
}

struct WtabParams {
  const double* cost;
  const double* mincost;
  double* wtab;
  u32* badcodes;
  u32* stats;
};

__global__ __launch_bounds__(256) void k_wtab(WtabParams P) {
  __shared__ u32 s_bad[40];
  const u32 b = blockIdx.x, tid = threadIdx.x;
  if (tid < 40) s_bad[tid] = 0;
  if (b == 0 && tid < 8 && P.stats) P.stats[tid] = 0;
  __syncthreads();
  const double* ll = P.cost + (u64)b * 320;
  const double* d = ll + 288;
  const double mincost = P.mincost[b];
  for (u32 c = tid; c < ZMX_WTAB; c += 256) {
    double w = __longlong_as_double(0x7ff0000000000000ll);
    if (c >= 1 && c <= 256) {
      w = ll[c - 1];
    } else if (c >= 257 && c < ZMX_NUM_W) {
      const u32 ls = 257u + (c - 257u) / 30u, ds = (c - 257u) % 30u;
      const int lb = ls < 265 || ls == 285 ? 0 : (int)(ls - 261) / 4;
      const int db = ds < 4 ? 0 : (int)ds / 2 - 1;
      w = ((double)(lb + db) + ll[ls]) + d[ds];
      if (w < mincost) {
        atomicAdd(&s_bad[0], 1u);
        atomicOr(&s_bad[4 + (c >> 5)], 1u << (c & 31));
      }
    }
    P.wtab[(u64)b * ZMX_WTAB + c] = w;
  }
  __syncthreads();
  if (tid < 40) P.badcodes[(u64)b * 40 + tid] = s_bad[tid];
}

struct BadScanParams {
  const BlockDesc* blocks;
  const u32* tile_off;
  u32 nb_total;
  const uint2* dph;
  const u16* codes;
  const u64* code_base;
  const u32* badcodes;
  u32* badpos;
};

__global__ __launch_bounds__(256) void k_badscan(BadScanParams P) {
  const u32 tile = blockIdx.x;
  const u32 b = find_block(P.tile_off, P.nb_total, tile);
  const u32* bad = P.badcodes + (u64)b * 40;
  if (bad[0] == 0) return;
  const BlockDesc bd = P.blocks[b];
  const u32 B = (u32)(bd.inend - bd.instart);
  const u32 tp0 = (tile - P.tile_off[b]) * MT;
  const u16* codes = P.codes + P.code_base[b];
  for (u32 p = tp0 + threadIdx.x; p < tp0 + MT && p < B; p += 256) {
    const uint2 dh = P.dph[bd.pos_off + p];
    const u32 kend = dh.y & 0xffffu;
    bool any = false;
    if (dh.y & DPH_CODELESS) {
      const u32 smax = (u32)(dev_length_symbol(kend) - 257);
      for (u32 sy = 0; sy <= smax; ++sy) {
        const u32 c = 257u + 30u * sy;
        any |= ((bad[4 + (c >> 5)] >> (c & 31)) & 1u) != 0;
      }
    } else {
      for (u32 k = 3; k <= kend; ++k) {
        const u32 c = (u32)codes[(u64)dh.x + k - 1] >> 3;
        any |= ((bad[4 + (c >> 5)] >> (c & 31)) & 1u) != 0;
      }
    }
    if (any) {
      const u64 gp = bd.pos_off + p;
      atomicOr(&P.badpos[gp >> 5], 1u << (gp & 31));
    }
  }
}

#define ZMX_PROF_N 56u
#define DP_RING 16384u
#define DP_PIECE 512u
#define DP_XN 704u
#define DP_FRONT 64u
#define DP_MIRROR 512u

#define DP_RELAX(CS, LS, WV, MCL)                                           \
  {                                                                         \
    const double old_ = (double)(CS);                                       \
    const double nc_ = (WV) + cj;                     \
    const bool upd_ = fmax(nc_, (MCL) + cj) < old_;                         \
    CS = upd_ ? (float)nc_ : CS;                                            \
    LS = upd_ ? src1 : LS;                                                  \
  }

__device__ __forceinline__ void dp_dma_piece(const u16* lane_src, u32 lds_byte_off) {
  lds_byte_off = (u32)__builtin_amdgcn_readfirstlane((int)lds_byte_off);
  u32 keep;
  asm volatile(
      "s_mov_b32 %0, m0\n\ts_mov_b32 m0, %2\n\ts_nop 0\n\tglobal_load_lds_dwordx4 %1, off\n\ts_mov_b32 m0, %0"
      : "=&s"(keep)
      : "v"(lane_src), "s"(lds_byte_off)
      : "memory");
}
```

### zopfli_amd/csrc/device/zmx_knobs.h

```cpp
#pragma once

#include <algorithm>
#include <cstdlib>

namespace zamd {

struct DeviceKnobs {
  bool guard = false;
  unsigned long long guard_selftest = 0;
  bool prof = false;
  bool kernel_timing = false;
  bool bc_prof = false;
  int match = 0;
  bool match_order = true;
  bool match_filter = true;
  unsigned long long match_hits = 300;
  unsigned long long pool_entries = 0;
  bool run_codes = false;
  unsigned long long code_budget_mb = 0;
  bool seg_l_set = false;
  unsigned seg_l = 4096;
  unsigned seg_head = 0;
  unsigned seg_warm = 512;
  unsigned seg_cuts = 1024;
  bool seg_mid = true;
  int seg_redo = 1;
  float seg_scale = 1.0f;
  int seg_debug = 0;
  int fix_lean = -1;
  int int_path = 1;
  int shortcut_chain = 1;
};

template <typename GetEnv>
DeviceKnobs ParseDeviceKnobs(GetEnv get) {
  auto clamped = [&](const char* name, unsigned dflt, unsigned lo, unsigned hi) {
    const char* e = get(name);
    if (!e) return dflt;
    const long v = std::atol(e);
    return v < static_cast<long>(lo) ? lo : v > static_cast<long>(hi) ? hi : static_cast<unsigned>(v);
  };
  auto integer = [&](const char* name, int dflt) { const char* e = get(name); return e ? std::atoi(e) : dflt; };
  auto on = [&](const char* name, bool dflt) { const char* e = get(name); return e ? std::atoi(e) != 0 : dflt; };
  auto count = [&](const char* name) { const char* e = get(name); return e ? static_cast<unsigned long long>(std::atoll(e)) : 0ull; };
  DeviceKnobs k;
  k.guard = on("ZOPFLI_AMD_GUARD", false);
  k.guard_selftest = count("ZOPFLI_AMD_GUARD_SELFTEST");
  k.prof = get("ZOPFLI_AMD_PROF") != nullptr;
  k.kernel_timing = on("ZOPFLI_AMD_KERNEL_TIMING", k.prof);
  k.bc_prof = get("ZOPFLI_AMD_BC_PROF") != nullptr;
  const int match = integer("ZOPFLI_AMD_MATCH", 0);
  k.match = match == 0 || match == 5 ? match : 2;
  k.match_order = on("ZOPFLI_AMD_MATCH_ORDER", true);
  k.match_filter = on("ZOPFLI_AMD_MATCH_FILTER", true);
  if (const char* e = get("ZOPFLI_AMD_MATCH_HITS")) k.match_hits = static_cast<unsigned long long>(std::max<long>(0, std::atol(e)));
  k.pool_entries = count("ZOPFLI_AMD_POOL_ENTRIES");
  k.run_codes = on("ZOPFLI_AMD_RUN_CODES", false);
  if (const char* e = get("ZOPFLI_AMD_CODE_BUDGET_MB")) k.code_budget_mb = static_cast<unsigned long long>(std::max<long>(1, std::atol(e)));
  k.seg_l_set = get("ZOPFLI_AMD_SEG_L") != nullptr;
  k.seg_l = clamped("ZOPFLI_AMD_SEG_L", 4096, 0, 1u << 24) & ~63u;
  k.seg_head = clamped("ZOPFLI_AMD_SEG_HEAD", 0, 0, 1u << 24) & ~63u;
  k.seg_warm = (clamped("ZOPFLI_AMD_SEG_WARM", 512, 64, 1u << 20) + 63u) & ~63u;
  k.seg_cuts = clamped("ZOPFLI_AMD_SEG_CUTS", 1024, 0, 1u << 16);
  k.seg_mid = clamped("ZOPFLI_AMD_SEG_MID", 1, 0, 1) != 0;
  k.seg_redo = integer("ZOPFLI_AMD_SEG_REDO", 1);
  if (const char* e = get("ZOPFLI_AMD_SEG_SCALE")) k.seg_scale = static_cast<float>(std::atof(e));
  k.seg_debug = integer("ZOPFLI_AMD_SEG_DEBUG", 0);
  k.fix_lean = integer("ZOPFLI_AMD_FIX_LEAN", -1);
  k.int_path = integer("ZOPFLI_AMD_INT_PATH", 1);
  k.shortcut_chain = integer("ZOPFLI_AMD_SHORTCUT_CHAIN", 1);
  return k;
}

inline const DeviceKnobs& Knobs() {
  static const DeviceKnobs k = ParseDeviceKnobs([](const char* name) -> const char* { return std::getenv(name); });
  return k;
}

}
```

### zopfli_amd/csrc/host/api.cc

```cpp
#include <chrono>
#include <malloc.h>
#include <cstdio>
#include <cstdlib>
#include <cstring>
#include <algorithm>
#include <condition_variable>
#include <memory>
#include <mutex>
#include <string>
#include <thread>
#include <unordered_map>
#include <vector>

#include "block_cache.h"
#include "block_cost.h"
#include "context_pool.h"
#include "deflate.h"
#include "lz77_optimal.h"
#include "symbols.h"
#include "deal.h"
#include "dealing.h"
#include "thread_pool.h"
#include "zmx_internal.h"
#include "zopfli_amd.h"

namespace zamd {

[[noreturn]] void Die(const char* what) {
  std::fprintf(stderr, "zopfli_amd: %s: %s\n", what, zmx_last_error());
  std::exit(EXIT_FAILURE);
}

void MaybeKeepHeap() {
  static const bool once = [] {
    const int mode = zamd::HostSwitches().keep_heap;
    if (mode == 0) return true;
    if (mode == 2) {
      mallopt(M_MMAP_THRESHOLD, 32 << 20);
      mallopt(M_TRIM_THRESHOLD, 1 << 30);
      mallopt(M_TOP_PAD, 64 << 20);
    } else {
      mallopt(M_TRIM_THRESHOLD, 1 << 30);
      mallopt(M_TOP_PAD, 256 << 20);
    }
    return true;
  }();
  (void)once;
}

zmx_stats& ThreadStats() {
  static thread_local zmx_stats stats = {};
  return stats;
}

}

namespace {

zmx_stats TakeStats() {
  const zmx_stats s = zamd::ThreadStats();
  zamd::ThreadStats() = zmx_stats{};
  return s;
}
void AddStats(const zmx_stats& s) {
  zmx_stats& t = zamd::ThreadStats();
  for (int i = 0; i < 3; ++i) t.kernel_seconds[i] += s.kernel_seconds[i];
  t.squeeze_launches += s.squeeze_launches;
  for (int i = 0; i < 3; ++i) t.match5[i] += s.match5[i];
  for (int i = 0; i < 4; ++i) t.match[i] += s.match[i];
  for (int i = 0; i < 8; ++i) t.seg[i] += s.seg[i];
}

using zamd::Die;
using zamd::kMasterBlock;
using zamd::Lease;
using zamd::MaybeKeepHeap;
using zamd::Pool;

bool TraceCall() { return zamd::HostSwitches().trace_call; }
double WallMs() {
  return std::chrono::duration<double, std::milli>(std::chrono::steady_clock::now().time_since_epoch()).count();
}

thread_local double g_traffic[3] = {0, 0, 0};
thread_local double g_out_traffic[4] = {0, 0, 0, 0};

#pragma weak zmx_internal_input_fetch
int FetchStoredBytes(zmx_ctx* ctx, std::vector<zamd::Chunk>* chunks, double* fetched) {
  for (zamd::Chunk& c : *chunks) {
    if (c.kind != zamd::Chunk::kStored || c.end == c.start) continue;
    if (!zmx_internal_input_fetch) {
      zmx_internal_set_error("stored block of a device input: this build cannot fetch its bytes", ZMX_ERR_DEVICE);
      return -1;
    }
    c.raw.resize(c.end - c.start);
    if (zmx_internal_input_fetch(ctx, c.start, c.end, c.raw.data()) != 0) return -1;
    *fetched += static_cast<double>(c.end - c.start);
  }
  return 0;
}

std::vector<zamd::Part> MasterBlocks(size_t insize, bool final) {
  std::vector<zamd::Part> parts;
  size_t i = 0;
  do {
    const bool masterfinal = i + kMasterBlock >= insize;
    const size_t size = masterfinal ? insize - i : kMasterBlock;
    parts.push_back({i, i + size, final && masterfinal});
    i += size;
  } while (i < insize);
  return parts;
}

int RunParts(zmx_ctx* ctx, const ZopfliOptions& options, int btype, const std::vector<zamd::Part>& parts,
             std::vector<zamd::Chunk>* chunks, std::vector<size_t>* part_chunks = nullptr, size_t group_bytes = 0) {
  size_t step = zamd::HostSwitches().parts_per_batch;
  size_t step_bytes = group_bytes;
  for (size_t a = 0; a < parts.size();) {
    size_t b = a + step < parts.size() ? a + step : parts.size();
    if (group_bytes) {
      b = a + 1;
      size_t bytes = parts[a].inend - parts[a].instart;
      while (b < parts.size() && b - a < 2048 && bytes + (parts[b].inend - parts[b].instart) <= step_bytes) {
        bytes += parts[b].inend - parts[b].instart;
        ++b;
      }
    }
    std::vector<zamd::Part> group(parts.begin() + static_cast<long>(a), parts.begin() + static_cast<long>(b));
    std::vector<zamd::Chunk> got;
    const int rc = zamd::DeflateParts(ctx, options, btype, group, &got, part_chunks);
    if (rc == -2 && b - a > 1) {
      step = (b - a + 1) / 2;
      step_bytes = std::max<size_t>(step_bytes / 2, 1);
      continue;
    }
    if (rc) return rc;
    for (auto& c : got) chunks->push_back(std::move(c));
    a = b;
  }
  return 0;
}

using zamd::ChecksumRequest;

struct Shard {
  size_t first = 0, last = 0, base = 0;
  std::vector<zamd::Chunk> chunks;
  std::vector<size_t> part_chunks;
  int rc = 0;
  std::string err;
  int err_class = ZMX_ERR_NONE;
  zamd::Timing timing;
  uint32_t sum = 0;
  size_t sum_bytes = 0;
  bool redone = false;
  zmx_stats stats = {};
  double traffic[3] = {0, 0, 0};
};

struct UploadOrder {
  std::mutex mu;
  std::condition_variable cv;
  std::vector<char> done;
  std::vector<long> after;
};
struct UploadTurn {
  UploadOrder& o; size_t d; bool released = false;
  void Wait() {
    if (o.after[d] < 0) return;
    std::unique_lock<std::mutex> lock(o.mu);
    o.cv.wait(lock, [&] { return o.done[static_cast<size_t>(o.after[d])] != 0; });
  }
  void Release() {
    if (released) return;
    released = true;
    { std::lock_guard<std::mutex> lock(o.mu); o.done[d] = 1; }
    o.cv.notify_all();
  }
  ~UploadTurn() { Release(); }
};

struct ShardedCall {
  const ZopfliOptions& options;
  int btype;
  const unsigned char* in;
  zamd::DeviceInput* dev;
  const std::vector<zamd::Part>& parts;
  ChecksumRequest* sum;
  bool want_part_chunks;
  zamd::ShardHooks* hooks;
  double t_begin;
  std::vector<Shard> shards;
  std::vector<int> priority;
  UploadOrder order;
};

size_t ContextsPerDevice(const ZopfliOptions& options, int btype, const unsigned char* in, const zamd::DeviceInput* dev,
                         const std::vector<zamd::Part>& parts, bool* runs) {
  const zamd::HostKnobs& k = zamd::HostSwitches();
  const size_t split_from = k.split_mb >= 0 ? static_cast<size_t>(k.split_mb) : (options.blocksplitting && btype == 2 ? 4 : 16);
  *runs = false;
  if (!split_from || parts.size() < split_from) return 1;
  *runs = dev ? dev->Runs()
              : in != nullptr && zamd::LooksLikeRuns(in, parts.front().instart, parts.back().inend);
  const bool one_context = *runs && !(k.stream_prio && k.split_runs);
  return one_context ? 1 : k.split_ways;
}

void PlanShards(ShardedCall* call, const std::vector<int>& device_of, bool runs) {
  const zamd::HostKnobs& k = zamd::HostSwitches();
  const std::vector<zamd::Part>& parts = call->parts;
  const size_t ndev = device_of.size();
  std::vector<double> cost;
  const bool have_costs = call->dev ? !call->dev->cost.empty() : call->in != nullptr;
  if (k.deal_by_cost && ndev > 1 && have_costs && parts.size() > ndev) {
    cost.resize(parts.size());
    if (call->dev) {
      for (size_t i = 0; i < parts.size(); ++i) cost[i] = call->dev->Cost(i);
    } else {
      zamd::ParallelFor(parts.size(), [&](size_t i) { cost[i] = zamd::MasterBlockCost(call->in, parts[i].instart, parts[i].inend); });
    }
  }
  const std::vector<size_t> first = zamd::ShardRanges(parts.size(), ndev, cost.empty() ? nullptr : cost.data(), k.shard_weights);
  call->shards = std::vector<Shard>(ndev);
  for (size_t d = 0; d < ndev; ++d) { call->shards[d].first = first[d]; call->shards[d].last = first[d + 1]; }
  const bool priorities = k.stream_prio && ((call->options.blocksplitting && call->btype == 2) || runs || k.stream_prio == 2);
  call->priority = priorities ? zamd::ShardPriorities(device_of) : std::vector<int>(ndev, 0);
  call->order.done.assign(ndev, 0);
  call->order.after = k.upload_order ? zamd::UploadAfter(device_of) : std::vector<long>(ndev, -1);
}

int SmallCallLevel(zmx_ctx* ctx) {
  static std::mutex mu;
  static std::unordered_map<zmx_ctx*, int> levels;
  std::lock_guard<std::mutex> g(mu);
  auto it = levels.find(ctx);
  if (it == levels.end()) it = levels.emplace(ctx, static_cast<int>(levels.size() % 3) - 1).first;
  return it->second;
}

void RunShard(ShardedCall* call, size_t d, zmx_ctx* ctx, bool retry) {
  const std::vector<zamd::Part>& parts = call->parts;
  zamd::ShardHooks* hooks = call->hooks;
  ChecksumRequest* sum = call->sum;
  Shard& sh = call->shards[d];
  UploadTurn turn{call->order, d};
  int level = retry ? 0 : call->priority[d];
  if (zamd::HostSwitches().small_prio && call->shards.size() == 1 && !retry) level = SmallCallLevel(ctx);
  if (zmx_ctx_set_priority(ctx, level) != 0) {
    std::fprintf(stderr, "zopfli_amd: stream priorities unavailable (%s)\n", zmx_last_error());
  }
  sh.rc = 0;
  sh.err.clear();
  sh.err_class = ZMX_ERR_NONE;
  sh.chunks.clear();
  sh.part_chunks.clear();
  sh.sum = 0;
  sh.sum_bytes = 0;
  auto fail = [&] { sh.rc = -1; sh.err = zmx_last_error(); sh.err_class = zmx_last_error_class(); };
  if (!retry && zamd::HostSwitches().test_fail_shard == static_cast<long>(d)) {
    sh.rc = -1;
    sh.err = "injected failure (ZOPFLI_AMD_TEST_FAIL_SHARD): PoolAlloc(pool) too large — the text must not matter";
    sh.err_class = ZMX_ERR_OUT_OF_MEMORY;
    return;
  }
  const size_t start = parts[sh.first].instart, end = parts[sh.last - 1].inend;
  sh.base = start > zamd::kWindow ? start - zamd::kWindow : 0;
  if (hooks) sh.base = std::max(sh.base, hooks->floor(parts[sh.first].instart));
  const double tr0 = WallMs();
  if (!retry) turn.Wait();
  const double tr1 = WallMs();
  const int up = call->dev ? call->dev->upload(ctx, sh.base, end - sh.base) : zmx_set_input(ctx, call->in + sh.base, end - sh.base);
  sh.traffic[call->dev ? 1 : 0] += static_cast<double>(end - sh.base);
  turn.Release();
  const double tr2 = WallMs();
  if (up != 0 || (hooks && hooks->uploaded(d, ctx, sh.base, sh.first, sh.last) != 0)) return fail();
  if (sum && start < sum->limit) {
    sh.sum_bytes = std::min(end, sum->limit) - start;
    if (zmx_checksum(ctx, sum->kind, start - sh.base, start - sh.base + sh.sum_bytes, &sh.sum) != 0) return fail();
  }
  std::vector<zamd::Part> mine(parts.begin() + static_cast<long>(sh.first), parts.begin() + static_cast<long>(sh.last));
  for (auto& p : mine) { p.instart -= sh.base; p.inend -= sh.base; }
  const double tr3 = WallMs();
  struct SplitOnDevice {
    bool was;
    explicit SplitOnDevice(bool on) : was(zamd::g_split_on_device) { zamd::g_split_on_device = on || was; }
    ~SplitOnDevice() { zamd::g_split_on_device = was; }
  } split_on_device(hooks && hooks->split_on_device);
  const bool device_output = call->dev && call->dev->device_output;
  struct DeviceOutput {
    bool was;
    explicit DeviceOutput(bool on) : was(zamd::g_device_output) { zamd::g_device_output = on; }
    ~DeviceOutput() { zamd::g_device_output = was; }
  } device_output_mode(device_output);
  sh.rc = RunParts(ctx, call->options, call->btype, mine, &sh.chunks, call->want_part_chunks ? &sh.part_chunks : nullptr,
                   hooks ? hooks->group_bytes : 0);
  if (!sh.rc && call->dev && !device_output && FetchStoredBytes(ctx,&sh.chunks, &sh.traffic[2]) != 0) sh.rc = -1;
  if (sh.rc) { sh.err = zmx_last_error(); sh.err_class = zmx_last_error_class(); }
  if (TraceCall()) {
    std::fprintf(stderr, "  shard %zu (%zu parts): start +%.2f ms, wait for turn %.2f, upload %.2f, checksum %.2f, parts %.2f, end +%.2f\n",
                 d, sh.last - sh.first, tr0 - call->t_begin, tr1 - tr0, tr2 - tr1, tr3 - tr2, WallMs() - tr3, WallMs() - call->t_begin);
  }
  for (auto& c : sh.chunks) {
    if (c.kind == zamd::Chunk::kStored) { c.start += sh.base; c.end += sh.base; }
  }
  sh.timing = zamd::ThreadTiming();
  if (d != 0 && !retry) sh.stats = TakeStats();
}

void RunShards(ShardedCall* call, const std::vector<zmx_ctx*>& ctxs) {
  const size_t ndev = call->shards.size();
  std::vector<std::thread> threads;
  for (size_t d = 1; d < ndev; ++d) threads.emplace_back(RunShard, call, d, ctxs[d], false);
  RunShard(call, 0, ctxs[0], false);
  for (auto& t : threads) t.join();
  for (size_t d = 1; d < ndev; ++d) AddStats(call->shards[d].stats);
  for (size_t d = 1; d < ndev; ++d) {
    const zamd::Timing& a = call->shards[d].timing;
    zamd::Timing& t = zamd::ThreadTiming();
    if (a.tables + a.greedy + a.squeeze + a.cost_model + a.split + a.encode >
        t.tables + t.greedy + t.squeeze + t.cost_model + t.split + t.encode) t = a;
  }
}

void RetryFailedShards(ShardedCall* call, const std::vector<zmx_ctx*>& ctxs) {
  std::vector<Shard>& shards = call->shards;
  for (size_t d = 0; d < shards.size(); ++d) {
    if (!shards[d].rc) continue;
    if (shards[d].err_class == ZMX_ERR_REFUSED) continue;
    zmx_ctx* other = nullptr;
    for (size_t e = 0; e < shards.size() && !other; ++e) if (e != d && !shards[e].rc && !shards[e].redone) other = ctxs[e];
    if (!other) break;
    std::fprintf(stderr, "zopfli_amd: a shard failed (%s): done again on another context\n", shards[d].err.c_str());
    RunShard(call, d, other, true);
    shards[d].redone = true;
  }
}

int CollectShards(ShardedCall* call, std::vector<zamd::Chunk>* chunks, std::vector<size_t>* part_chunks) {
  for (auto& sh : call->shards) {
    if (sh.rc) {
      std::fprintf(stderr, "zopfli_amd: device error: %s\n", sh.err.c_str());
      if (call->hooks) { call->hooks->error = sh.err; call->hooks->error_class = sh.err_class; }
      if (call->dev) { call->dev->error = sh.err; call->dev->error_class = sh.err_class; }
      return sh.rc;
    }
    for (auto& c : sh.chunks) chunks->push_back(std::move(c));
    if (part_chunks) part_chunks->insert(part_chunks->end(), sh.part_chunks.begin(), sh.part_chunks.end());
  }
  return 0;
}

struct InlineHostWork {
  bool on, was;
  explicit InlineHostWork(bool o) : on(o), was(zamd::g_host_inline) { if (on) zamd::g_host_inline = true; }
  ~InlineHostWork() { if (on) zamd::g_host_inline = was; }
};

int RunPartsShardedOnce(const ZopfliOptions& options, int btype, const unsigned char* in,
                        const std::vector<zamd::Part>& parts, std::vector<zamd::Chunk>* chunks,
                        ChecksumRequest* sum = nullptr, std::vector<size_t>* part_chunks = nullptr,
                        zamd::ShardHooks* hooks = nullptr, zamd::DeviceInput* dev = nullptr) {
  bool runs = false;
  const size_t per_device = ContextsPerDevice(options, btype, in, dev, parts, &runs);
  const double tr_begin = WallMs();
  const Lease lease(parts.size(), per_device, parts.size() < 32, parts.size() < 32, dev ? dev->only_device : -1);
  if (lease.ctxs.empty()) {
    dev->error = "device " + std::to_string(dev->only_device) + " is not one of the library's devices (ZOPFLI_AMD_DEVICE, ZOPFLI_AMD_DEVICES)";
    dev->error_class = ZMX_ERR_REFUSED;
    return -1;
  }
  const double tr_lease = WallMs();
  const InlineHostWork inline_host(parts.size() <= 2 && Pool().InFlight() > 1);
  const size_t ndev = std::min(lease.ctxs.size(), parts.size());
  ShardedCall call{options, btype, in, dev, parts, sum, part_chunks != nullptr, hooks, tr_begin, {}, {}, {}};
  PlanShards(&call, std::vector<int>(lease.device_of.begin(), lease.device_of.begin() + static_cast<long>(ndev)), runs);
  RunShards(&call, lease.ctxs);
  RetryFailedShards(&call, lease.ctxs);
  for (const Shard& sh : call.shards) for (int i = 0; i < 3; ++i) g_traffic[i] += sh.traffic[i];
  const double tr_joined = WallMs();
  const int rc = CollectShards(&call, chunks, part_chunks);
  if (rc) {
    for (zamd::Chunk& c : *chunks) c.dev_owner.reset();
    return rc;
  }
  if (TraceCall()) {
    std::fprintf(stderr, "RunPartsSharded: lease %.2f ms, shards done +%.2f, chunks moved +%.2f\n", tr_lease - tr_begin,
                 tr_joined - tr_begin, WallMs() - tr_begin);
  }
  if (sum) {
    sum->value = sum->kind == ZMX_ADLER32 ? 1u : 0u;
    for (auto& sh : call.shards) {
      if (sh.sum_bytes) sum->value = zmx_checksum_combine(sum->kind, sum->value, sh.sum, sh.sum_bytes);
    }
  }
  if (dev && dev->finish) {
    const int frc = dev->finish(lease.ctxs[0], chunks, sum ? sum->value : 0);
    if (frc) { dev->error = zmx_last_error(); dev->error_class = zmx_last_error_class(); }
    for (zamd::Chunk& c : *chunks) c.dev_owner.reset();
    return frc;
  }
  return 0;
}

int RunPartsSharded(const ZopfliOptions& options, int btype, const unsigned char* in,
                    const std::vector<zamd::Part>& parts, std::vector<zamd::Chunk>* chunks,
                    ChecksumRequest* sum = nullptr, zamd::DeviceInput* dev = nullptr) {
  const size_t round_parts = zamd::HostSwitches().round_parts;
  if (dev) dev->first_part = 0;
  if (parts.size() <= round_parts) return RunPartsShardedOnce(options, btype, in, parts, chunks, sum, nullptr, nullptr, dev);
  uint32_t acc = sum ? (sum->kind == ZMX_ADLER32 ? 1u : 0u) : 0u;
  for (size_t a = 0; a < parts.size(); a += round_parts) {
    const size_t b = std::min(parts.size(), a + round_parts);
    if (dev) dev->first_part = a;
    const std::vector<zamd::Part> round(parts.begin() + static_cast<long>(a), parts.begin() + static_cast<long>(b));
    ChecksumRequest rs{sum ? sum->kind : 0, sum ? sum->limit : 0, 0};
    const int rc = RunPartsShardedOnce(options, btype, in, round, chunks, sum ? &rs : nullptr, nullptr, nullptr, dev);
    if (rc) return rc;
    if (sum && round.front().instart < sum->limit) {
      const size_t covered = std::min(round.back().inend, sum->limit) - round.front().instart;
      acc = zmx_checksum_combine(sum->kind, acc, rs.value, covered);
    }
  }
  if (sum) sum->value = acc;
  return 0;
}

void EmitChunks(const std::vector<zamd::Chunk>& chunks, const unsigned char* in, unsigned char* bp,
                unsigned char** out, size_t* outsize, bool verbose = false) {
  const size_t before = *outsize;
  zamd::MergeChunks(chunks, in, bp, out, outsize, verbose);
  g_out_traffic[0] += static_cast<double>(*outsize - before);
}

void ResetTiming() {
  zamd::ThreadTiming() = zamd::Timing();
  (void)TakeStats();
  g_traffic[0] = g_traffic[1] = g_traffic[2] = 0;
  for (double& t : g_out_traffic) t = 0;
}

void PushByte(unsigned v, unsigned char** out, size_t* outsize) {
  const uint8_t b = static_cast<uint8_t>(v);
  zamd::AppendToOutput(&b, 1, out, outsize);
}

}

namespace zamd {
std::vector<Part> InputMasterBlocks(size_t insize, bool final) { return MasterBlocks(insize, final); }
int RunPartsDealt(const ZopfliOptions& options, int btype, const unsigned char* in, const std::vector<Part>& parts,
                  std::vector<Chunk>* chunks, std::vector<size_t>* part_chunks, ShardHooks* hooks, DeviceInput* dev) {
  return RunPartsShardedOnce(options, btype, in, parts, chunks, nullptr, part_chunks, hooks, dev);
}
void ResetCallStats() { ResetTiming(); }
void AddDeviceTraffic(double bytes) { g_traffic[1] += bytes; }
void SetOutputTraffic(const double* t4) { for (int i = 0; i < 4; ++i) g_out_traffic[i] = t4[i]; }
int RunPartsToDevice(const ZopfliOptions& options, const std::vector<Part>& parts, ChecksumRequest* sum, DeviceInput* dev) {
  std::vector<Chunk> chunks;
  return RunPartsShardedOnce(options, 2, nullptr, parts, &chunks, sum, nullptr, nullptr, dev);
}
bool TraceCallOn() { return TraceCall(); }
double CallWallMs() { return WallMs(); }
int OnPooledContext(const std::function<int(zmx_ctx*)>& fn, int only_device) {
  Lease lease(1, 1, false, false, only_device);
  if (lease.ctxs.empty()) {
    const std::string msg = "device " + std::to_string(only_device) + " is not one of the library's devices (ZOPFLI_AMD_DEVICE, ZOPFLI_AMD_DEVICES)";
    zmx_internal_set_error(msg.c_str(), ZMX_ERR_REFUSED);
    return -1;
  }
  return fn(lease.ctxs[0]);
}
}

extern "C" {

size_t zmx_host_cache_trim(void) { return zamd::BlockCache::Trim(); }

void ZopfliInitOptions(ZopfliOptions* options) {
  options->verbose = 0;
  options->verbose_more = 0;
  options->numiterations = 15;
  options->blocksplitting = 1;
  options->blocksplittinglast = 0;
  options->blocksplittingmax = 15;
}

void ZopfliDeflatePart(const ZopfliOptions* options, int btype, int final, const unsigned char* in,
                       size_t instart, size_t inend, unsigned char* bp, unsigned char** out,
                       size_t* outsize) {
  ResetTiming();
  std::vector<zamd::Part> parts{{instart, inend, final != 0}};
  std::vector<zamd::Chunk> chunks;
  if (RunPartsSharded(*options, btype, in, parts, &chunks) != 0) Die("device error");
  EmitChunks(chunks, in, bp, out, outsize, options->verbose != 0);
}

}

namespace {
struct Input {
  const unsigned char* in;
  zamd::DeviceInput* dev;
};

int DeflateWhole(const ZopfliOptions* options, int btype, int final, const Input& input, size_t insize,
                 const unsigned char* prefix, size_t nprefix, unsigned char* bp, unsigned char** out, size_t* outsize,
                 ChecksumRequest* sum) {
  const unsigned char* in = input.in;
  const size_t offset = *outsize + nprefix;
  {
    const double tr0 = WallMs();
    ResetTiming();
    const std::vector<zamd::Part> parts = MasterBlocks(insize, final != 0);
    std::vector<zamd::Chunk> chunks;
    const double tr1 = WallMs();
    if (const int rc = RunPartsSharded(*options, btype, in, parts, &chunks, sum, input.dev)) return rc;
    const double tr2 = WallMs();
    if (nprefix) zamd::AppendToOutput(prefix, nprefix, out, outsize);
    g_out_traffic[0] += static_cast<double>(nprefix);
    EmitChunks(chunks, in, bp, out, outsize, options->verbose != 0);
    const double tr3 = WallMs();
    chunks.clear();
    chunks.shrink_to_fit();
    if (TraceCall()) {
      std::fprintf(stderr, "DeflateWhole: set-up %.2f ms, parts %.2f, merge %.2f, chunks freed %.2f\n", tr1 - tr0, tr2 - tr1,
                   tr3 - tr2, WallMs() - tr3);
    }
// ... 227 lines not shown
```

### zopfli_amd/csrc/host/zmx_internal.h

```cpp
#pragma once
#include <cstddef>
#include <cstdint>

#include "zopfli_amd.h"

#define ZMX_INTERNAL_EXPORT __attribute__((visibility("default")))

struct zmx_stats {
  double kernel_seconds[3];
  double squeeze_launches;
  double match5[3];
  double match[4];
  double seg[8];
};
namespace zamd {
zmx_stats& ThreadStats();
}

extern "C" {

void zmx_internal_set_error(const char* msg, int cls);

int zmx_internal_device(zmx_ctx* ctx);
size_t zmx_internal_input_size(zmx_ctx* ctx);
const unsigned char* zmx_internal_input_host(zmx_ctx* ctx);
int zmx_internal_input_fetch(zmx_ctx* ctx, size_t begin, size_t end, unsigned char* dst);
int zmx_internal_probe_counts(zmx_ctx* ctx, const void* bytes, size_t n, const uint64_t* ranges, uint32_t* counts);
ZMX_INTERNAL_EXPORT void zmx_internal_pool_stats(zmx_ctx* ctx, uint64_t out[8]);

int zmx_internal_device_pointer(const char* who, const void* p, size_t n, int* device);
int zmx_internal_device_pointers(const char* who, size_t n, const void* const* p, const size_t* nbytes);
int zmx_internal_device_alloc(int device, size_t n, void** p);
void zmx_internal_device_free(int device, void* p);

int zmx_internal_bitjoin_literals(zmx_ctx* ctx, const unsigned char* literals, size_t nliterals, size_t n, zmx_bit_piece* pieces,
                                  const unsigned char* is_literal, uint64_t total_bits, void* d_dst, size_t dst_capacity);
int zmx_internal_bitjoin_many_literals(zmx_ctx* ctx, const unsigned char* literals, size_t nliterals, size_t ndst, const zmx_bit_dest* dests,
                                       const size_t* capacity, size_t npieces, zmx_bit_piece* pieces, const unsigned char* is_literal);
int zmx_internal_device_pointers_one_device(const char* who, size_t n, const void* const* p, const size_t* nbytes, int* device);

int zmx_internal_png_scanlines(zmx_ctx* ctx, const void* d_image, size_t linebytes, size_t height, size_t bytewidth, int strategy,
                               unsigned windowsize, const unsigned char* predefined, void* d_out);

int zmx_internal_png_reduced_scanlines(zmx_ctx* ctx, const zmx_png_image* image, const zmx_png_color_mode* mode, int strategy,
                                       unsigned windowsize, const unsigned char* predefined, void* d_out);

ZMX_INTERNAL_EXPORT double zmx_internal_gather_ms(void);
ZMX_INTERNAL_EXPORT double zmx_internal_bitjoin_ms(void);
ZMX_INTERNAL_EXPORT double zmx_internal_png_rows_ms(void);
ZMX_INTERNAL_EXPORT void zmx_internal_png_color_ms(double out[3]);
ZMX_INTERNAL_EXPORT void zmx_internal_run_info(const double* cost320, float* wmax, uint32_t* tiemask);

}
```

Before: 866.3 MB/s.

## Pack redo tasks into full workgroups and recheck only touched boundaries

The redo pass now packs up to four failing segment tasks into each workgroup instead of one task per workgroup, and it runs on a capped grid. A new recheck kernel verifies only the boundaries next to redone tasks rather than relaunching a full check over every task. Workgroup task lists are rebuilt as compact descriptors, with an optional pull-based stretch kernel that lets a workgroup work through more tasks than it has waves. SegL also uses the per-device position count under sharding, and extra profiling counters are added. The aim is to cut idle waves and launch-wide rescans during redo, at the cost of extra atomics and more complex bookkeeping.

```diff
diff --git a/zopfli_amd/csrc/device/drv_build.h b/zopfli_amd/csrc/device/drv_build.h
--- a/zopfli_amd/csrc/device/drv_build.h
+++ b/zopfli_amd/csrc/device/drv_build.h
@@ -6,6 +6,7 @@
 extern "C" {
 static unsigned SegL(u64 total_positions) {
   if (Knobs().seg_l_set) return Knobs().seg_l;
+  total_positions = std::max<u64>(total_positions, zamd::CallPositions());
   return total_positions <= (128u << 10) ? 256u : total_positions <= (16u << 20) ? 512u : total_positions <= (48u << 20) ? 1024u : 2048u;
 }
 static unsigned SegHead(size_t nb) {
@@ -543,7 +544,8 @@
   HIPCHK(PoolAlloc(c, &t->d_mid, nt));
   HIPCHK(PoolAlloc(c, &t->d_chk, nt));
   HIPCHK(PoolAlloc(c, &t->d_over, nt * SEG_OVER));
-  HIPCHK(PoolAlloc(c, &t->d_redo, 4 + nt * 4));
+  t->redo_cap = nt;
+  HIPCHK(PoolAlloc(c, &t->d_redo, 4 + nt * 4 + nt * 2));
   HIPCHK(hipMemcpyAsync(t->d_tasks, t->tasks.data(), nt * sizeof(SegTask), hipMemcpyHostToDevice, c->stream));
   HIPCHK(hipMemcpyAsync(t->d_task_off, t->task_off.data(), (nb + 1) * sizeof(u32), hipMemcpyHostToDevice, c->stream));
   HIPCHK(hipMemsetAsync(t->run.stats(t->d_runout), 0, RunLayout::kStats * sizeof(u32), c->stream));
@@ -623,27 +625,36 @@
     HIPCHK(hipMemcpyAsync(kind.data(), d_kind, ntk * sizeof(u32), hipMemcpyDeviceToHost, c->stream));
     HIPCHK(hipStreamSynchronize(c->stream));
   }
-  std::vector<u32> wg, wg_runs;
-  for (int pass = 0; pass < 2; ++pass) {
-    for (size_t b = 0; b < nb; ++b) {
-      const u32 a0 = t->task_off[b], a1 = t->task_off[b + 1];
-      std::vector<u32> grp[2];
-      for (u32 k = a0; k < a1; ++k) grp[kind[k] ? 1 : 0].push_back(k);
-      for (int kd = 0; kd < 2; ++kd) {
-        std::vector<u32>& dst = kd ? wg_runs : wg;
-        for (size_t i = 0; i < grp[kd].size(); i += D5_WG) {
-          const bool has_head = i == 0 && !grp[kd].empty() && grp[kd][0] == a0;
-          if ((pass == 0) != has_head) continue;
-          for (u32 w = 0; w < D5_WG; ++w) dst.push_back(i + w < grp[kd].size() ? grp[kd][i + w] : SEG_NONE);
-        }
+  const u32 S = Knobs().seg_stretch;
+  std::vector<u32> list[2];
+  std::vector<uint2> desc[2][2];
+  for (size_t b = 0; b < nb; ++b) {
+    const u32 a0 = t->task_off[b], a1 = t->task_off[b + 1];
+    for (int kd = 0; kd < 2; ++kd) {
+      const u32 l0 = static_cast<u32>(list[kd].size());
+      for (u32 k = a0; k < a1; ++k)
+        if ((kind[k] ? 1 : 0) == kd) list[kd].push_back(k);
+      const u32 l1 = static_cast<u32>(list[kd].size());
+      for (u32 i = l0; i < l1; i += S) {
+        const bool has_head = i == l0 && list[kd][l0] == a0;
+        desc[kd][has_head ? 0 : 1].push_back(make_uint2(i, std::min(S, l1 - i)));
       }
     }
   }
-  t->n_wg = static_cast<u32>(wg.size() / D5_WG);
-  t->n_wg_runs = static_cast<u32>(wg_runs.size() / D5_WG);
-  wg.insert(wg.end(), wg_runs.begin(), wg_runs.end());
-  HIPCHK(PoolAlloc(c, &t->d_wg_tasks, wg.size() + 4));
-  if (!wg.empty()) HIPCHK(hipMemcpyAsync(t->d_wg_tasks, wg.data(), wg.size() * sizeof(u32), hipMemcpyHostToDevice, c->stream));
+  const u32 shift = static_cast<u32>(list[0].size());
+  std::vector<uint2> wg;
+  for (int kd = 0; kd < 2; ++kd)
+    for (int rest = 0; rest < 2; ++rest)
+      for (uint2 d : desc[kd][rest]) wg.push_back(make_uint2(d.x + (kd ? shift : 0u), d.y));
+  t->n_wg = static_cast<u32>(desc[0][0].size() + desc[0][1].size());
+  t->n_wg_runs = static_cast<u32>(desc[1][0].size() + desc[1][1].size());
+  list[0].insert(list[0].end(), list[1].begin(), list[1].end());
+  HIPCHK(PoolAlloc(c, &t->d_wg_tasks, list[0].size() + 4));
+  HIPCHK(PoolAlloc(c, &t->d_wg_desc, wg.size() + 1));
+  if (!wg.empty()) {
+    HIPCHK(hipMemcpyAsync(t->d_wg_tasks, list[0].data(), list[0].size() * sizeof(u32), hipMemcpyHostToDevice, c->stream));
+    HIPCHK(hipMemcpyAsync(t->d_wg_desc, wg.data(), wg.size() * sizeof(uint2), hipMemcpyHostToDevice, c->stream));
+  }
   HIPCHK(hipStreamSynchronize(c->stream));
   return 0;
 }
@@ -712,6 +723,9 @@
   cp.wg_tasks = t->d_wg_tasks;
   cp.redo_count = t->d_redo;
   cp.redo_wg = t->d_redo + 4;
+  cp.recheck = t->d_redo + 4 + t->redo_cap * 4;
+  cp.redo_parity = 0;
+  cp.wg_desc = t->d_wg_desc;
   cp.flags = t->run.flags(t->d_runout);
   cp.wmeta = t->d_wmeta;
   cp.winroff = t->d_winroff;
diff --git a/zopfli_amd/csrc/device/drv_squeeze.h b/zopfli_amd/csrc/device/drv_squeeze.h
--- a/zopfli_amd/csrc/device/drv_squeeze.h
+++ b/zopfli_amd/csrc/device/drv_squeeze.h
@@ -107,6 +107,11 @@
     for (size_t b = 0; b < nb; ++b) { mx = std::max(mx, static_cast<double>(pr[b * ZMX_PROF_N + 7])); hd = std::max(hd, static_cast<double>(pr[b * ZMX_PROF_N + 8])); }
     std::fprintf(stderr, "  k_dp5_spec: longest task %.0f cycles, longest head task %.0f cycles; %.1f%% of the positions walked by the integer step (cycles per position there: fetch issue %.1f, fetch wait %.1f, gather + chain %.1f)\n", mx, hd, 100.0 * a[10] / (a[4] + 1e-9), a[11] / (a[10] + 1e-9), a[12] / (a[10] + 1e-9), a[13] / (a[10] + 1e-9));
   }
+  if (a[56] > 0 && a[57] > 0) {
+    std::fprintf(stderr, "  k_dp5_spec fixed cost: set-up %.0f cycles a wave (%.0f waves with a task), %.2f%% of the workgroups' wave cycles; finished waves waiting for their workgroup %.2f%%; in tasks %.2f%%\n",
+                 a[54] / a[56], a[56], 100.0 * a[54] / a[57], 100.0 * a[55] / a[57], 100.0 * a[1] / a[57]);
+  }
+  std::fprintf(stderr, "  redo list: %.0f tasks in %.0f entries\n", a[58], a[59]);
   std::fprintf(stderr, "  k_dp5_spec integer windows, cycles per position: class decision %.1f, waiting for the prefetched record and codes %.1f, prefetch issue %.1f\n",
                a[20] / (a[10] + 1e-9), a[21] / (a[10] + 1e-9), a[22] / (a[10] + 1e-9));
   std::fprintf(stderr, "  k_dp5_spec windows: integer %.1f%% of positions at %.0f cycles each, class 1 in doubles %.1f%% at %.0f, class 2 %.1f%% at %.0f, generic %.1f%% at %.0f\n",
@@ -160,9 +165,19 @@
   return 0;
 }
 
+constexpr unsigned kRedoGrid = 1024;
 static void LaunchSpec(hipStream_t stream, unsigned grid, bool run_tasks, const Dp4Params& p) {
   const dim3 g(grid), b(64 * D5_WG);
-  if (run_tasks) {
+  const bool pull = p.redo_pass ? p.redo_pack > 1 : Knobs().seg_stretch > D5_WG || Knobs().seg_pull;
+  if (pull) {
+    if (run_tasks) {
+      if (p.prof) hipLaunchKernelGGL((k_dp5_stretch<true, 2, true>), g, b, 0, stream, p);
+      else hipLaunchKernelGGL((k_dp5_stretch<false, 2, true>), g, b, 0, stream, p);
+    } else {
+      if (p.prof) hipLaunchKernelGGL((k_dp5_stretch<true, 4, false>), g, b, 0, stream, p);
+      else hipLaunchKernelGGL((k_dp5_stretch<false, 4, false>), g, b, 0, stream, p);
+    }
+  } else if (run_tasks) {
     if (p.prof) hipLaunchKernelGGL((k_dp5_spec<true, 2, true>), g, b, 0, stream, p);
     else hipLaunchKernelGGL((k_dp5_spec<false, 2, true>), g, b, 0, stream, p);
   } else {
@@ -253,15 +268,17 @@
       hipLaunchKernelGGL(k_dpcheck, dim3(ntask), dim3(64), 0, c->stream, cp);
       KCHK(c, "k_dpcheck");
       for (int pass = 0; pass < knobs.seg_redo; ++pass) {
-        hipLaunchKernelGGL(k_dpscan, dim3(nblk), dim3(64), 0, c->stream, cp);
-        KCHK(c, "k_dpscan");
         Dp4Params c2 = cp;
         c2.redo_pass = 1;
         c2.est_bits = nullptr;
-        LaunchSpec(c->stream, ntask, t->n_wg_runs != 0, c2);
-        KCHK(c, "k_dp5_spec");
-        hipLaunchKernelGGL(k_dpcheck, dim3(ntask), dim3(64), 0, c->stream, cp);
-        KCHK(c, "k_dpcheck");
+        c2.redo_parity = pass & 1;
+        c2.redo_pack = t->n_wg_runs != 0 ? 1 : 4;
+        hipLaunchKernelGGL(k_dpscan, dim3(nblk), dim3(64), 0, c->stream, c2);
+        KCHK(c, "k_dpscan");
+        LaunchSpec(c->stream, c2.redo_pack > 1 ? std::min(ntask, kRedoGrid) : ntask, t->n_wg_runs != 0, c2);
+        KCHK(c, "k_dp5_spec (redo)");
+        hipLaunchKernelGGL(k_dprecheck, dim3(std::min(ntask, DPRECHECK_GRID)), dim3(64), 0, c->stream, c2);
+        KCHK(c, "k_dprecheck");
       }
       LaunchFix(c->stream, nblk, cp);
       KCHK(c, "k_dp4_fix");
diff --git a/zopfli_amd/csrc/device/drv_tables.h b/zopfli_amd/csrc/device/drv_tables.h
--- a/zopfli_amd/csrc/device/drv_tables.h
+++ b/zopfli_amd/csrc/device/drv_tables.h
@@ -86,6 +86,7 @@
   SegTask* d_tasks = nullptr;
   u32* d_task_off = nullptr;
   u32* d_wg_tasks = nullptr;
+  uint2* d_wg_desc = nullptr;
   u32 n_wg = 0;
   u32 n_wg_runs = 0;
   u32* d_wmeta = nullptr;
@@ -100,6 +101,7 @@
   SegCheck* d_chk = nullptr;
   u16* d_over = nullptr;
   u32* d_redo = nullptr;
+  size_t redo_cap = 0;
   std::vector<u32> h_hist;
   bool have_hist = false;
   u32 squeeze_runs = 0;
@@ -114,7 +116,7 @@
   rel(t->d_blocks, t->d_tile_off, t->d_same16, t->d_links, t->d_recs, t->d_pool, t->d_la, t->d_dph, t->d_block_edges);
   rel(t->d_badpos, t->d_code_base, t->d_codes, t->d_wtab, t->d_badcodes, t->d_seg_off, t->d_extab, t->d_seginfo);
   rel(t->d_counters, t->d_prof, t->d_tasks, t->d_task_off, t->d_wg_tasks, t->d_wmeta, t->d_runin, t->d_runout);
-  rel(t->d_winroff, t->d_winflag, t->d_win_off, t->d_lvl, t->d_entry, t->d_exit, t->d_mid, t->d_chk, t->d_over, t->d_redo);
+  rel(t->d_winroff, t->d_winflag, t->d_win_off, t->d_lvl, t->d_entry, t->d_exit, t->d_mid, t->d_chk, t->d_over, t->d_redo, t->d_wg_desc);
   PinnedGive(c, &t->h_runin, t->h_runin_cap);
   PinnedGive(c, &t->h_runout, t->h_runout_cap);
   t->params = TableParams{};
diff --git a/zopfli_amd/csrc/device/zmx_dp4.h b/zopfli_amd/csrc/device/zmx_dp4.h
--- a/zopfli_amd/csrc/device/zmx_dp4.h
+++ b/zopfli_amd/csrc/device/zmx_dp4.h
@@ -254,6 +254,7 @@
   u32* stats;
   float level_scale;
   const u32* wg_tasks;
+  const uint2* wg_desc;
   const u32* wmeta;
   const u32* winroff;
   const u32* winflag;
@@ -262,6 +263,9 @@
   u16* over;
   u32* redo_count;
   u32* redo_wg;
+  u32* recheck;
+  int redo_pack;
+  int redo_parity;
   int int_path;
   int fix_lean_min;
   int redo_pass;
@@ -791,11 +795,23 @@
 }
 
 __global__ __launch_bounds__(64) void k_dpcheck(Dp4Params P) {
-  if (blockIdx.x == 0 && threadIdx.x == 0) *P.redo_count = 0;
+  if (blockIdx.x == 0 && threadIdx.x < 3) P.redo_count[threadIdx.x] = 0;
   const u32 t = P.task0 + blockIdx.x;
   if (P.tasks[t].pout == 0) return;
   const SegCheck r = d4_check(&P.exit[t - 1], &P.entry[t], threadIdx.x);
   if (threadIdx.x == 0) P.chk[t] = r;
+}
+
+#define DPRECHECK_GRID 1024u
+__global__ __launch_bounds__(64) void k_dprecheck(Dp4Params P) {
+  if (blockIdx.x == 0 && threadIdx.x == 0) { P.redo_count[0] = 0; P.redo_count[2 - P.redo_parity] = 0; }
+  const u32 n = P.redo_count[1 + P.redo_parity];
+  for (u32 i = blockIdx.x; i < n; i += gridDim.x) {
+    const u32 t = P.recheck[i];
+    if (P.tasks[t].pout == 0) continue;
+    const SegCheck r = d4_check(&P.exit[t - 1], &P.entry[t], threadIdx.x);
+    if (threadIdx.x == 0) P.chk[t] = r;
+  }
 }
 
 __device__ __forceinline__ u32 d4_accept(float vmin, double vmax, double delta, double wmax, u32 tiemask) {
@@ -814,6 +830,7 @@
   const double wmax = (double)P.wmax[b] + 1.0;
   const u32 tiemask = P.tiemask[b];
   double carry = 0.0;
+  u32 cur = 0, fill = 0;
   for (u32 c0 = t0 + 1; c0 < t1; c0 += 64) {
     const u32 t = c0 + lane;
     const bool act = t < t1;
@@ -828,17 +845,44 @@
       if ((int)lane >= o) incl += up;
     }
     const double delta = carry + incl;
-    if (act) {
-      const bool ok = ck.match == 1 && d4_accept(ck.vmin, (double)vmax, delta, wmax, tiemask) == 0;
-      if (!ok && ck.match != 0) {
-        const u32 slot = atomicAdd(P.redo_count, 1u);
-        u32* wg = P.redo_wg + (u64)slot * 4;
+    const bool again = act && ck.match != 0 && !(ck.match == 1 && d4_accept(ck.vmin, (double)vmax, delta, wmax, tiemask) == 0);
+    const u64 m = __ballot(again);
+    if (m && P.prof && lane == 0) atomicAdd(&P.prof[(u64)b * ZMX_PROF_N + 58], (u64)__popcll(m));
+    if (m && P.redo_pack == 1) {
+      if (P.prof && lane == 0) atomicAdd(&P.prof[(u64)b * ZMX_PROF_N + 59], (u64)__popcll(m));
+      if (again) {
+        u32* wg = P.redo_wg + (u64)atomicAdd(&P.redo_count[0], 1u) * 4;
         wg[0] = t; wg[1] = SEG_NONE; wg[2] = SEG_NONE; wg[3] = SEG_NONE;
         P.lvl[t] = (float)((double)P.lvl[t] + delta);
-      }
+        const u32 k = atomicAdd(&P.redo_count[1 + P.redo_parity], t + 1 < t1 ? 2u : 1u);
+        P.recheck[k] = t;
+        if (t + 1 < t1) P.recheck[k + 1] = t + 1;
+      }
+    } else if (m) {
+      const u32 n = (u32)__popcll(m);
+      const u32 fresh = (fill + n + 3u) / 4u - (fill ? 1u : 0u);
+      u32 base = 0;
+      if (fresh && lane == 0) base = atomicAdd(&P.redo_count[0], fresh);
+      base = (u32)__builtin_amdgcn_readfirstlane((int)base);
+      if (fresh && P.prof && lane == 0) atomicAdd(&P.prof[(u64)b * ZMX_PROF_N + 59], (u64)fresh);
+      const u32 first = fill ? cur : base;
+      const u32 after = fill ? base : base + 1u;
+      if (again) {
+        const u32 r = fill + (u32)__popcll(m & ((1ull << lane) - 1ull));
+        const u32 e = r < 4u ? first : after + (r >> 2) - 1u;
+        P.redo_wg[(u64)e * 4 + (r & 3u)] = t;
+        P.lvl[t] = (float)((double)P.lvl[t] + delta);
+        const u32 k = atomicAdd(&P.redo_count[1 + P.redo_parity], t + 1 < t1 ? 2u : 1u);
+        P.recheck[k] = t;
+        if (t + 1 < t1) P.recheck[k + 1] = t + 1;
+      }
+      const u32 tot = fill + n;
+      cur = tot <= 4u ? first : after + ((tot + 3u) >> 2) - 2u;
+      fill = tot & 3u;
     }
     carry += __shfl(incl, 63, 64);
   }
+  if (fill && lane >= fill && lane < 4u) P.redo_wg[(u64)cur * 4 + lane] = SEG_NONE;
 }
 
 __device__ __forceinline__ void d4_copy_over(const Dp4Params& P, u32 t, u32 B, u16* la) {
diff --git a/zopfli_amd/csrc/device/zmx_dp5.h b/zopfli_amd/csrc/device/zmx_dp5.h
--- a/zopfli_amd/csrc/device/zmx_dp5.h
+++ b/zopfli_amd/csrc/device/zmx_dp5.h
@@ -1057,7 +1057,6 @@
 }
 
 #define D5_WG 4u
-#define FIX_CH 256u
 template <bool PROF, int WAVES, bool RUNS>
 __global__ __launch_bounds__(64 * D5_WG, WAVES) void k_dp5_spec(Dp4Params P) {
   __shared__ __align__(16) double s_wtab[ZMX_WTAB];
@@ -1068,15 +1067,32 @@
   __shared__ __align__(8) uint2 s_ri[D5_WG][32];
   __shared__ __align__(8) uint2 s_rk[RUNS ? D5_WG : 1u][RUNS ? D5_RKN : 1u];
   __shared__ u32 s_rmax;
+  __shared__ unsigned long long s_pf_sum, s_pf_max;
+  __shared__ u32 s_pf_done;
+  const u64 t_wg0 = PROF ? (u64)__builtin_readcyclecounter() : 0ull;
   const u32 wave = (u32)__builtin_amdgcn_readfirstlane((int)(threadIdx.x >> 6));
   if (P.redo_pass && blockIdx.x >= *P.redo_count) return;
-  const u32* wg = (P.redo_pass ? P.redo_wg : P.wg_tasks) + (u64)(P.task0 + blockIdx.x) * D5_WG;
+  const uint2 wd = P.redo_pass ? make_uint2(0u, 1u) : P.wg_desc[P.task0 + blockIdx.x];
+  const u32* wg = P.redo_pass ? P.redo_wg + (u64)blockIdx.x * D5_WG : P.wg_tasks + wd.x;
   const u32 t0 = wg[0];
   const u32 b0 = P.tasks[t0].block;
   for (u32 i = threadIdx.x; i < ZMX_WTAB; i += 64 * D5_WG) s_wtab[i] = P.wtab[(u64)b0 * ZMX_WTAB + i];
-  if (threadIdx.x == 0) s_rmax = 0;
+  if (threadIdx.x == 0) { s_rmax = 0; if (PROF) { s_pf_sum = 0; s_pf_max = 0; s_pf_done = 0; } }
   __syncthreads();
   d5_build_w1(s_wtab, s_w1, s_sym1);
+  auto prof_done = [&]() {
+    if (PROF && P.prof && (threadIdx.x & 63u) == 0) {
+      const unsigned long long te = (unsigned long long)((u64)__builtin_readcyclecounter() - t_wg0);
+      atomicAdd(&s_pf_sum, te);
+      atomicMax(&s_pf_max, te);
+      __builtin_amdgcn_fence(__ATOMIC_ACQ_REL, "workgroup");
+      if (atomicAdd(&s_pf_done, 1u) == D5_WG - 1u) {
+        __builtin_amdgcn_fence(__ATOMIC_ACQ_REL, "workgroup");
+        atomicAdd(&P.prof[(u64)b0 * ZMX_PROF_N + 55], (u64)(D5_WG * s_pf_max - s_pf_sum));
+        atomicAdd(&P.prof[(u64)b0 * ZMX_PROF_N + 57], (u64)(D5_WG * s_pf_max));
+      }
+    }
+  };
   auto task_level = [&](u32 tt) -> float {
     const SegTask K = P.tasks[tt];
     float lv = P.est_bits ? P.est_bits[K.block] * ((float)K.q / (float)(u32)(P.blocks[K.block].inend - P.blocks[K.block].instart)) : P.lvl[tt];
@@ -1086,7 +1102,7 @@
   D5IntTab IT;
   IT.on = false; IT.lo = 0; IT.span = 0;
   {
-    const u32 tl = P.tasks[t0].pout != 0 ? t0 : wg[1];
+    const u32 tl = P.tasks[t0].pout != 0 ? t0 : wd.y > 1u ? wg[1] : SEG_NONE;
     if (tl != SEG_NONE && P.int_path) {
       const u32 lb = __float_as_uint(task_level(tl));
       const int e = (int)(lb >> 23) - 127;
@@ -1100,12 +1116,12 @@
       }
     }
   }
+  if (wave >= wd.y) { prof_done(); return; }
   const u32 t = wg[wave];
-  if (t == SEG_NONE) return;
   const SegTask T = P.tasks[t];
   const BlockDesc bd = P.blocks[T.block];
   const u32 B = (u32)(bd.inend - bd.instart);
-  if (B == 0) return;
+  if (B == 0) { prof_done(); return; }
   D4Job J;
   J.start = T.q & ~31u;
   J.cell = T.q & 31u;
@@ -1130,10 +1146,167 @@
     J.level = task_level(t);
     if (P.est_bits && (threadIdx.x & 63) == 0) P.lvl[t] = J.level;
   }
+  if (PROF && P.prof && (threadIdx.x & 63u) == 0) {
+    atomicAdd(&P.prof[(u64)b0 * ZMX_PROF_N + 54], (u64)__builtin_readcyclecounter() - t_wg0);
+    atomicAdd(&P.prof[(u64)b0 * ZMX_PROF_N + 56], 1ull);
+  }
   d5_run_job<PROF, RUNS>(P, J, T.block, bd, s_wtab, reinterpret_cast<float*>(s_buf[wave]), reinterpret_cast<u16*>(s_buf[wave] + 4u * DP_XN),
                    reinterpret_cast<u16*>(s_buf[wave]), s_itab, IT, s_w1, s_sym1, s_ri[wave], s_rk[RUNS ? wave : 0u]);
+  prof_done();
 }
 
+#define D5_STRETCH_MAX 32u
+template <bool PROF, int WAVES, bool RUNS>
+__global__ __launch_bounds__(64 * D5_WG, WAVES) void k_dp5_stretch(Dp4Params P) {
+  __shared__ __align__(16) double s_wtab[ZMX_WTAB];
+  __shared__ __align__(16) unsigned char s_buf[D5_WG][D5_STAGE_BYTES];
+  __shared__ __align__(8) uint2 s_itab[ZMX_WTAB];
+  __shared__ __align__(8) double s_w1[D5_W1];
+  __shared__ u8 s_sym1[D5_W1];
+  __shared__ __align__(8) uint2 s_ri[D5_WG][32];
+  __shared__ __align__(8) uint2 s_rk[RUNS ? D5_WG : 1u][RUNS ? D5_RKN : 1u];
+  __shared__ u32 s_rmax;
+  __shared__ u32 s_next;
+  __shared__ u32 s_hdr[4];
+  __shared__ u32 s_tid[D5_STRETCH_MAX];
+  __shared__ __align__(16) SegTask s_task[D5_STRETCH_MAX];
+  __shared__ float s_lvl[D5_STRETCH_MAX];
+  __shared__ unsigned long long s_pf_sum, s_pf_max;
+  __shared__ u32 s_pf_done;
+  const u32 wave = (u32)__builtin_amdgcn_readfirstlane((int)(threadIdx.x >> 6));
+  const u32 lane = threadIdx.x & 63u;
+  u32 item = P.redo_pass ? blockIdx.x : P.task0 + blockIdx.x;
+  const u32 n_items = P.redo_pass ? *P.redo_count : item + 1u;
+  for (; item < n_items; item += gridDim.x) {
+    const u64 t_wg0 = PROF ? (u64)__builtin_readcyclecounter() : 0ull;
+    const u32* list;
+    u32 count = 0;
+    if (P.redo_pass) {
+      list = P.redo_wg + (u64)item * D5_WG;
+      while (count < D5_WG && list[count] != SEG_NONE) ++count;
+    } else {
+      const uint2 d = P.wg_desc[item];
+      list = P.wg_tasks + d.x;
+      count = d.y < D5_STRETCH_MAX ? d.y : D5_STRETCH_MAX;
+    }
+    if (count == 0) continue;
+    const u32 b0 = P.tasks[list[0]].block;
+    const BlockDesc bd = P.blocks[b0];
+    const u32 B = (u32)(bd.inend - bd.instart);
+    for (u32 i = threadIdx.x; i < ZMX_WTAB; i += 64 * D5_WG) s_wtab[i] = P.wtab[(u64)b0 * ZMX_WTAB + i];
+    for (u32 i = threadIdx.x; i < count; i += 64 * D5_WG) {
+      const u32 tt = list[i];
+      const SegTask K = P.tasks[tt];
+      float lv = 0.0f;
+      if (K.pout != 0) {
+        lv = P.est_bits ? P.est_bits[b0] * ((float)K.q / (float)B) : P.lvl[tt];
+        if (!P.redo_pass) lv *= P.level_scale;
+        lv = lv >= 16.0f ? lv : 16.0f;
+        if (P.est_bits) P.lvl[tt] = lv;
+      }
+      s_tid[i] = tt;
+      s_task[i] = K;
+      s_lvl[i] = lv;
+    }
+    if (threadIdx.x == 0) { s_rmax = 0; s_next = 0; if (PROF) { s_pf_sum = 0; s_pf_max = 0; s_pf_done = 0; } }
+    __syncthreads();
+    d5_build_w1(s_wtab, s_w1, s_sym1);
+    {
+      const u32 il = s_task[0].pout != 0 ? 0u : 1u;
+      bool on = false;
+      u32 lb = 0;
+      if (il < count && P.int_path) {
+        lb = __float_as_uint(s_lvl[il]);
+        const int e = (int)(lb >> 23) - 127;
+        if (e >= 4 && e < 31 && ((P.tiemask[b0] >> (e & 31)) & 1u) == 0) {
+          d5_build_inttab(s_wtab, s_itab, s_rmax, e);
+          on = true;
+        }
+      }
+      if (threadIdx.x == 0) { s_hdr[0] = b0; s_hdr[1] = B != 0 ? count : 0u; s_hdr[2] = on ? 1u : 0u; s_hdr[3] = lb & 0x7f800000u; }
+      __syncthreads();
+    }
+    bool first_job = true;
+    for (;;) {
+      u32 i = 0;
+      if (lane == 0) i = atomicAdd(&s_next, 1u);
+      i = (u32)__builtin_amdgcn_readfirstlane((int)i);
+      if (i >= (u32)__builtin_amdgcn_readfirstlane((int)s_hdr[1])) break;
+      typedef const __attribute__((address_space(4))) unsigned char* kargp;
+      kargp kq = (kargp)__builtin_amdgcn_kernarg_segment_ptr();
+      asm volatile("" : "+s"(kq));
+      Dp4Params Pj = P;
+#define D5_KARG(F) Pj.F = *reinterpret_cast<const __attribute__((address_space(4))) decltype(Dp4Params::F)*>(kq + offsetof(Dp4Params, F));
+      D5_KARG(blocks) D5_KARG(dph) D5_KARG(cost) D5_KARG(mincost) D5_KARG(codes) D5_KARG(code_base) D5_KARG(la) D5_KARG(prof)
+      D5_KARG(badpos) D5_KARG(entry) D5_KARG(exit) D5_KARG(mid) D5_KARG(wmax) D5_KARG(tiemask) D5_KARG(wmeta) D5_KARG(winroff)
+      D5_KARG(winflag) D5_KARG(win_off) D5_KARG(over) D5_KARG(int_path) D5_KARG(chain_fast) D5_KARG(debug) D5_KARG(flags)
+#undef D5_KARG
+      const Dp4Params& P = Pj;
+      const u32 b0 = (u32)__builtin_amdgcn_readfirstlane((int)s_hdr[0]);
+      const BlockDesc bd = P.blocks[b0];
+      const u32 B = (u32)(bd.inend - bd.instart);
+      D5IntTab IT;
+      IT.on = __builtin_amdgcn_readfirstlane((int)s_hdr[2]) != 0;
+      IT.lo = (u32)__builtin_amdgcn_readfirstlane((int)s_hdr[3]);
+      {
+        const u32 rm = (u32)__builtin_amdgcn_readfirstlane((int)s_rmax);
+        IT.span = !IT.on ? 0u : rm < 0x100000u ? 33u * rm : 0x40000000u;
+      }
+      const u32 t = (u32)__builtin_amdgcn_readfirstlane((int)s_tid[i]);
+      SegTask T;
+      T.block = b0;
+      T.q = (u32)__builtin_amdgcn_readfirstlane((int)s_task[i].q);
+      T.pout = (u32)__builtin_amdgcn_readfirstlane((int)s_task[i].pout);
+      T.pend = (u32)__builtin_amdgcn_readfirstlane((int)s_task[i].pend);
+      D4Job J;
+      J.start = T.q & ~31u;
+      J.cell = T.q & 31u;
+      J.noshort = 0;
+      J.pout = T.pout;
+      J.pend = T.pend;
+      J.load = false;
+      J.delta = 0;
+      J.init = nullptr;
+      J.entry = &P.entry[t];
+      J.exit = &P.exit[t];
+      J.mid = T.pout != 0 && P.mid != nullptr ? &P.mid[t] : nullptr;
+      J.over_lo = T.pend <= B ? T.pend : SEG_NONE;
+      J.over = P.over + (u64)t * SEG_OVER;
+      if (T.pout == 0) {
+        J.spec = false;
+        J.la_lo = 1;
+        J.level = 0.0f;
+      } else {
+        J.spec = true;
+        J.la_lo = SEG_NONE;
+        J.level = __uint_as_float((u32)__builtin_amdgcn_readfirstlane((int)__float_as_uint(s_lvl[i])));
+      }
+      if (PROF && P.prof && first_job && lane == 0) {
+        atomicAdd(&P.prof[(u64)b0 * ZMX_PROF_N + 54], (u64)__builtin_readcyclecounter() - t_wg0);
+        atomicAdd(&P.prof[(u64)b0 * ZMX_PROF_N + 56], 1ull);
+      }
+      first_job = false;
+      d5_run_job<PROF, RUNS>(P, J, b0, bd, s_wtab, reinterpret_cast<float*>(s_buf[wave]), reinterpret_cast<u16*>(s_buf[wave] + 4u * DP_XN),
+                       reinterpret_cast<u16*>(s_buf[wave]), s_itab, IT, s_w1, s_sym1, s_ri[wave], s_rk[RUNS ? wave : 0u]);
+      asm volatile("s_waitcnt vmcnt(0) lgkmcnt(0)" ::: "memory");
+    }
+    if (PROF && P.prof && lane == 0) {
+      const unsigned long long te = (unsigned long long)((u64)__builtin_readcyclecounter() - t_wg0);
+      atomicAdd(&s_pf_sum, te);
+      atomicMax(&s_pf_max, te);
+      __builtin_amdgcn_fence(__ATOMIC_ACQ_REL, "workgroup");
+      if (atomicAdd(&s_pf_done, 1u) == D5_WG - 1u) {
+        __builtin_amdgcn_fence(__ATOMIC_ACQ_REL, "workgroup");
+        atomicAdd(&P.prof[(u64)b0 * ZMX_PROF_N + 55], (u64)(D5_WG * s_pf_max - s_pf_sum));
+        atomicAdd(&P.prof[(u64)b0 * ZMX_PROF_N + 57], (u64)(D5_WG * s_pf_max));
+      }
+    }
+    if (!P.redo_pass) return;
+    __syncthreads();
+  }
+}
+
+#define FIX_CH 256u
 template <bool PROF>
 __global__ __launch_bounds__(64 * (D3_NB + 2)) void k_dp4_fix(Dp4Params P) {
   D4_LDS_DECL
diff --git a/zopfli_amd/csrc/device/zmx_kernels.h b/zopfli_amd/csrc/device/zmx_kernels.h
--- a/zopfli_amd/csrc/device/zmx_kernels.h
+++ b/zopfli_amd/csrc/device/zmx_kernels.h
@@ -572,7 +572,7 @@
   }
 }
 
-#define ZMX_PROF_N 56u
+#define ZMX_PROF_N 60u
 #define DP_RING 16384u
 #define DP_PIECE 512u
 #define DP_XN 704u
diff --git a/zopfli_amd/csrc/device/zmx_knobs.h b/zopfli_amd/csrc/device/zmx_knobs.h
--- a/zopfli_amd/csrc/device/zmx_knobs.h
+++ b/zopfli_amd/csrc/device/zmx_knobs.h
@@ -24,6 +24,8 @@
   unsigned seg_warm = 512;
   unsigned seg_cuts = 1024;
   bool seg_mid = true;
+  unsigned seg_stretch = 4;
+  bool seg_pull = false;
   int seg_redo = 1;
   float seg_scale = 1.0f;
   int seg_debug = 0;
@@ -63,6 +65,8 @@
   k.seg_warm = (clamped("ZOPFLI_AMD_SEG_WARM", 512, 64, 1u << 20) + 63u) & ~63u;
   k.seg_cuts = clamped("ZOPFLI_AMD_SEG_CUTS", 1024, 0, 1u << 16);
   k.seg_mid = clamped("ZOPFLI_AMD_SEG_MID", 1, 0, 1) != 0;
+  k.seg_stretch = clamped("ZOPFLI_AMD_SEG_STRETCH", 4, 1, 32);
+  k.seg_pull = on("ZOPFLI_AMD_SEG_PULL", false);
   k.seg_redo = integer("ZOPFLI_AMD_SEG_REDO", 1);
   if (const char* e = get("ZOPFLI_AMD_SEG_SCALE")) k.seg_scale = static_cast<float>(std::atof(e));
   k.seg_debug = integer("ZOPFLI_AMD_SEG_DEBUG", 0);
diff --git a/zopfli_amd/csrc/host/api.cc b/zopfli_amd/csrc/host/api.cc
--- a/zopfli_amd/csrc/host/api.cc
+++ b/zopfli_amd/csrc/host/api.cc
@@ -51,6 +51,11 @@
 zmx_stats& ThreadStats() {
   static thread_local zmx_stats stats = {};
   return stats;
+}
+
+unsigned long long& CallPositions() {
+  static thread_local unsigned long long positions = 0;
+  return positions;
 }
 
 }
@@ -192,6 +197,7 @@
   double t_begin;
   std::vector<Shard> shards;
   std::vector<int> priority;
+  std::vector<unsigned long long> device_positions;
   UploadOrder order;
 };
 
@@ -224,6 +230,12 @@
   const std::vector<size_t> first = zamd::ShardRanges(parts.size(), ndev, cost.empty() ? nullptr : cost.data(), k.shard_weights);
   call->shards = std::vector<Shard>(ndev);
   for (size_t d = 0; d < ndev; ++d) { call->shards[d].first = first[d]; call->shards[d].last = first[d + 1]; }
+  call->device_positions.assign(ndev, 0);
+  for (size_t d = 0; d < ndev && !runs; ++d) {
+    for (size_t e = 0; e < ndev; ++e) {
+      if (device_of[e] == device_of[d] && first[e + 1] > first[e]) call->device_positions[d] += parts[first[e + 1] - 1].inend - parts[first[e]].instart;
+    }
+  }
   const bool priorities = k.stream_prio && ((call->options.blocksplitting && call->btype == 2) || runs || k.stream_prio == 2);
   call->priority = priorities ? zamd::ShardPriorities(device_of) : std::vector<int>(ndev, 0);
   call->order.done.assign(ndev, 0);
@@ -282,6 +294,10 @@
   std::vector<zamd::Part> mine(parts.begin() + static_cast<long>(sh.first), parts.begin() + static_cast<long>(sh.last));
   for (auto& p : mine) { p.instart -= sh.base; p.inend -= sh.base; }
   const double tr3 = WallMs();
+  struct CallPositionsScope {
+    explicit CallPositionsScope(unsigned long long n) { zamd::CallPositions() = n; }
+    ~CallPositionsScope() { zamd::CallPositions() = 0; }
+  } call_positions(call->shards.size() > 1 ? call->device_positions[d] : 0);
   struct SplitOnDevice {
     bool was;
     explicit SplitOnDevice(bool on) : was(zamd::g_split_on_device) { zamd::g_split_on_device = on || was; }
@@ -373,7 +389,7 @@
   const double tr_lease = WallMs();
   const InlineHostWork inline_host(parts.size() <= 2 && Pool().InFlight() > 1);
   const size_t ndev = std::min(lease.ctxs.size(), parts.size());
-  ShardedCall call{options, btype, in, dev, parts, sum, part_chunks != nullptr, hooks, tr_begin, {}, {}, {}};
+  ShardedCall call{options, btype, in, dev, parts, sum, part_chunks != nullptr, hooks, tr_begin, {}, {}, {}, {}};
   PlanShards(&call, std::vector<int>(lease.device_of.begin(), lease.device_of.begin() + static_cast<long>(ndev)), runs);
   RunShards(&call, lease.ctxs);
   RetryFailedShards(&call, lease.ctxs);
diff --git a/zopfli_amd/csrc/host/zmx_internal.h b/zopfli_amd/csrc/host/zmx_internal.h
--- a/zopfli_amd/csrc/host/zmx_internal.h
+++ b/zopfli_amd/csrc/host/zmx_internal.h
@@ -15,6 +15,7 @@
 };
 namespace zamd {
 zmx_stats& ThreadStats();
+unsigned long long& CallPositions();
 }
 
 extern "C" {
```

Result: faster. 932.1 MB/s, median of 6 (+7.6%).
